# tczhangzhi/pytorch-distributed

Measured on NVIDIA H100. Metric: ResNet-50 images/sec (device-timed, max over ranks), higher is better.
Workload: dtype bf16; 1 GPU; model=resnet50, global_batch=256, image_size=224, parallelism=dp1, entry=distributed, comm=fused, nvls=False, channels_last=True, fused_bn=True, optimizer=fused, cuda_graph=True, l2_policy=inputs larger than L2 (4 x 38.5 MB bf16 batches + GBs of activations per step), overlap_optimizer=True, bucket_view=False, cudnn=deterministic

## Files before the change

### pytorch_distributed_b200/_ext.py

```python
from __future__ import annotations

import hashlib
import importlib.util
import os
import shutil
import sys
import threading

_HERE = os.path.dirname(os.path.abspath(__file__))
_CSRC = os.path.join(_HERE, "csrc")
_NAME = "_C"
_SO = os.path.join(_HERE, _NAME + ".so")
_STAMP = os.path.join(_HERE, _NAME + ".hash")
_SOURCES = ["bindings.cpp", "symm.cpp", "hvd_core.cpp", "collectives.cu", "optim.cu", "bn_act.cu", "data_ops.cu", "gemm_bnstats.cu", "stem_conv.cu",
            "resample.cu"]
_lock = threading.Lock()
_mod = None
_err = None

CUDA_FLAGS = ["-gencode", "arch=compute_90a,code=sm_90a", "-lineinfo", "-O3", "--use_fast_math", "-std=c++17",
              "--expt-relaxed-constexpr", "-Xptxas", "-v"]


def source_hash() -> str:
    h = hashlib.sha256()
    for fn in sorted(os.listdir(_CSRC)):
        if fn.endswith((".cu", ".cpp", ".h", ".cuh")):
            with open(os.path.join(_CSRC, fn), "rb") as f:
                h.update(fn.encode())
                h.update(f.read())
    h.update(" ".join(CUDA_FLAGS).encode())
    return h.hexdigest()


def is_built() -> bool:
    if not (os.path.exists(_SO) and os.path.exists(_STAMP)):
        return False
    with open(_STAMP) as f:
        return f.read().strip() == source_hash()


def build(verbose: bool = False, force: bool = False) -> str:
    with _lock:
        if is_built() and not force:
            return _SO
        from torch.utils import cpp_extension
        build_dir = os.path.join(_CSRC, "build")
        os.makedirs(build_dir, exist_ok=True)
        os.environ.setdefault("MAX_JOBS", str(max(2, min(8, (os.cpu_count() or 4)))))
        cpp_extension.load(
            name=_NAME,
            sources=[os.path.join(_CSRC, s) for s in _SOURCES],
            extra_cflags=["-O3", "-std=c++17"],
            extra_cuda_cflags=CUDA_FLAGS,
            extra_include_paths=[_CSRC],
            build_directory=build_dir,
            verbose=verbose,
            is_python_module=False,
        )
        built = os.path.join(build_dir, _NAME + ".so")
        shutil.copyfile(built, _SO + ".tmp")
        os.replace(_SO + ".tmp", _SO)
        with open(_STAMP, "w") as f:
            f.write(source_hash())
        return _SO


def _import_so():
    import torch
    spec = importlib.util.spec_from_file_location("pytorch_distributed_b200." + _NAME, _SO)
    mod = importlib.util.module_from_spec(spec)
    spec.loader.exec_module(mod)
    sys.modules["pytorch_distributed_b200." + _NAME] = mod
    return mod


def lib(build_if_missing: bool = True):
    global _mod, _err
    if _mod is not None:
        return _mod
    if _err is not None:
        raise _err
    try:
        if not is_built():
            if not build_if_missing or os.environ.get("PTD_NO_BUILD") == "1":
                raise RuntimeError("native extension is not built (run `python -c 'import __graft_entry__ as g; g.build()'`)")
            build()
        _mod = _import_so()
        return _mod
    except Exception as e:
        _err = RuntimeError("pytorch_distributed_b200 native extension unavailable: %s" % (e,))
        raise _err from e


def available() -> bool:
    try:
        lib()
        return True
    except Exception:
        return False


def require_on_cuda() -> None:
    import torch
    if torch.cuda.is_available():
        lib()


launches = 0


def note_launch(n: int = 1) -> None:
    global launches
    launches += n
```

### pytorch_distributed_b200/csrc/bindings.cpp

```cpp
#include <torch/extension.h>

#include "hvd_core.h"
#include "host.h"
#include "symm.h"

namespace py = pybind11;
using namespace ptd;

namespace {

at::Tensor arena_view(const std::shared_ptr<SymmArena>& a, int64_t rank, int64_t offset_bytes, int64_t numel, const std::string& dtype) {
  at::ScalarType st;
  if (dtype == "float32") st = at::kFloat;
  else if (dtype == "bfloat16") st = at::kBFloat16;
  else if (dtype == "float16") st = at::kHalf;
  else if (dtype == "int32") st = at::kInt;
  else if (dtype == "uint8") st = at::kByte;
  else throw std::runtime_error("unsupported arena view dtype " + dtype);
  const int64_t esz = (int64_t)c10::elementSize(st);
  TORCH_CHECK(offset_bytes >= 0 && offset_bytes + numel * esz <= a->bytes(), "arena view out of range");
  TORCH_CHECK(offset_bytes % esz == 0, "misaligned arena view");
  const int r = a->single_process() ? (int)rank : a->rank();
  void* p = reinterpret_cast<void*>(a->ptr(r) + offset_bytes);
  auto keep = a;
  return at::from_blob(p, {numel}, [keep](void*) {}, at::TensorOptions().dtype(st).device(at::kCUDA, (c10::DeviceIndex)a->device(r)));
}

}

PYBIND11_MODULE(TORCH_EXTENSION_NAME, m) {
  m.doc() = "pytorch_distributed_b200 native runtime (sm_90a)";
  m.attr("MAX_WORLD") = kMaxWorld;
  m.attr("MAX_BLOCKS") = kMaxBlocks;
  m.attr("MAX_CHANNELS") = kMaxChannels;
  m.attr("MAX_PTRS") = kMaxPtrs;
  m.attr("SIGNAL_PAD_BYTES") = (int64_t)sizeof(SignalPad);
  m.attr("SEG_BYTES") = (int64_t)sizeof(Seg);
  m.def("multicast_supported", &multicast_supported);

  py::class_<SymmArena, std::shared_ptr<SymmArena>>(m, "SymmArena")
      .def(py::init<int, int, int, int64_t>(), py::arg("device"), py::arg("rank"), py::arg("world"), py::arg("bytes"))
      .def_static("create_local", &SymmArena::create_local)
      .def_static("from_pointers", &SymmArena::from_pointers)
      .def("export_fd", &SymmArena::export_fd)
      .def("open_socket", &SymmArena::open_socket)
      .def("send_fd", &SymmArena::send_fd)
      .def("recv_fd", &SymmArena::recv_fd, py::call_guard<py::gil_scoped_release>())
      .def("map_peer", &SymmArena::map_peer)
      .def("mc_create", &SymmArena::mc_create)
      .def("mc_import", &SymmArena::mc_import)
      .def("mc_add_device", &SymmArena::mc_add_device)
      .def("mc_bind_and_map", &SymmArena::mc_bind_and_map)
      .def("disable_multicast", &SymmArena::disable_multicast)
      .def_property_readonly("rank", &SymmArena::rank)
      .def_property_readonly("world", &SymmArena::world)
      .def_property_readonly("bytes", &SymmArena::bytes)
      .def_property_readonly("mc_ptr", &SymmArena::mc_ptr)
      .def_property_readonly("multicast_candidate", &SymmArena::multicast_candidate)
      .def_property_readonly("has_multicast", &SymmArena::has_multicast)
      .def_property_readonly("mc_error", &SymmArena::mc_error)
      .def_property_readonly("single_process", &SymmArena::single_process)
      .def("ptr", &SymmArena::ptr)
      .def("device", &SymmArena::device, py::arg("r") = 0)
      .def("status", &SymmArena::status)
      .def("set_timeout_ms", &SymmArena::set_timeout_ms)
      .def("ll_seq_ptr", &SymmArena::ll_seq_ptr, py::arg("r") = 0)
      .def("view", [](std::shared_ptr<SymmArena> a, int64_t offset, int64_t numel, const std::string& dtype, int64_t rank) {
             return arena_view(a, rank, offset, numel, dtype);
           }, py::arg("offset_bytes"), py::arg("numel"), py::arg("dtype"), py::arg("rank") = 0)
      .def("launch_plan",
           [](std::shared_ptr<SymmArena> a, int channel, int as_rank, int kind, int wire_dtype, bool nvls, int grid, std::vector<at::Tensor> tensors,
              int64_t seg_begin_ptr, int64_t segs_ptr, int64_t data_off_bytes, int64_t block_elems, int64_t plan_calls_ptr, int64_t found_inf_ptr,
              double scale, bool writeback, int root, int flags, int64_t result_off_bytes) {
             launch_plan(a->ctx(channel, as_rank), kind, wire_dtype, nvls, grid, tensors, seg_begin_ptr, segs_ptr, data_off_bytes, block_elems,
                         plan_calls_ptr, found_inf_ptr, scale, writeback, root, flags, result_off_bytes);
           },
           py::arg("channel"), py::arg("as_rank"), py::arg("kind"), py::arg("wire_dtype"), py::arg("nvls"), py::arg("grid"), py::arg("tensors"),
           py::arg("seg_begin_ptr"), py::arg("segs_ptr"), py::arg("data_off_bytes"), py::arg("block_elems"), py::arg("plan_calls_ptr"),
           py::arg("found_inf_ptr"), py::arg("scale"), py::arg("writeback"), py::arg("root"), py::arg("flags") = 0,
           py::arg("result_off_bytes") = (int64_t)-1)
      .def("launch_barrier", [](std::shared_ptr<SymmArena> a, int channel) { launch_barrier(a->ctx(channel)); })
      .def("launch_metrics",
           [](std::shared_ptr<SymmArena> a, int channel, const at::Tensor& logits, const at::Tensor& target, c10::optional<at::Tensor> loss, at::Tensor out) {
             launch_metrics(a->ctx(channel), logits, target, loss, a->ll_seq_ptr(), out);
           })
      .def("launch_ll_allreduce", [](std::shared_ptr<SymmArena> a, int channel, const at::Tensor& in, at::Tensor out, double scale) {
        launch_ll_allreduce(a->ctx(channel), in, out, scale, a->ll_seq_ptr());
      });

  m.def("pack_pointers", &pack_pointers);
  m.def("fused_sgd_flat", &fused_sgd_flat, py::arg("grad"), py::arg("master"), py::arg("momentum"), py::arg("model_copy"), py::arg("hyper"),
        py::arg("found_inf"), py::arg("nesterov"), py::arg("first_step"));
  m.def("fused_sgd_multi", &fused_sgd_multi);
  m.def("multi_tensor_scale", &multi_tensor_scale);
  m.def("multi_tensor_axpby", &multi_tensor_axpby);
  m.def("amp_update_scale", &amp_update_scale);
  m.def("bn_act_forward", &bn_act_forward);
  m.def("bn_act_backward", &bn_act_backward);
  m.def("bn_act_backward2", &bn_act_backward2);
  m.def("stem_forward", &stem_forward);
  m.def("stem_forward_pre", &stem_forward_pre);
  m.def("stem_backward", &stem_backward);
  m.def("stem_im2col", &stem_im2col);
  m.def("conv1x1_bnstats", &conv1x1_bnstats);
  m.def("normalize_nhwc", &normalize_nhwc);
  m.def("resample_normalize", &resample_normalize, py::arg("arena"), py::arg("n"), py::arg("out_h"), py::arg("out_w"), py::arg("max_rows"),
        py::arg("a"), py::arg("b"), py::arg("out_dtype"), py::arg("channels_last"));
  m.def("p2p_copy_multi", &p2p_copy_multi);

  py::class_<FusionQueue, std::shared_ptr<FusionQueue>>(m, "FusionQueue")
      .def(py::init<int64_t, double, int64_t>(), py::arg("fusion_threshold_bytes"), py::arg("cycle_time_ms"), py::arg("cycle_bytes") = 0)
      .def("wait_idle", &FusionQueue::wait_idle, py::arg("timeout_ms"), py::call_guard<py::gil_scoped_release>())
      .def("wake", &FusionQueue::wake)
      .def("set_cycle_bytes", &FusionQueue::set_cycle_bytes)
      .def("cycle_bytes", &FusionQueue::cycle_bytes)
      .def("enable_timeline", &FusionQueue::enable_timeline)
      .def("timeline", &FusionQueue::timeline)
      .def("enqueue", &FusionQueue::enqueue, py::arg("name"), py::arg("nbytes"), py::arg("order_key"))
      .def("next_group", &FusionQueue::next_group, py::arg("timeout_ms"), py::call_guard<py::gil_scoped_release>())
      .def("flush", &FusionQueue::flush)
      .def("mark_done", &FusionQueue::mark_done)
      .def("wait", &FusionQueue::wait, py::arg("handle"), py::arg("timeout_ms"), py::call_guard<py::gil_scoped_release>())
      .def("pending", &FusionQueue::pending)
      .def("shutdown", &FusionQueue::shutdown)
      .def("stats", &FusionQueue::stats);
}
```

### pytorch_distributed_b200/csrc/bn_act.cu

```cuda
#include <ATen/cuda/CUDAContext.h>
#include <c10/cuda/CUDAGuard.h>
#include <torch/extension.h>

#include <map>

#include "common.cuh"
#include "host.h"

namespace ptd {

constexpr int kBnThreads = 256;
constexpr int kBnWarps = kBnThreads / 32;

struct RowMap {
  int cgs;
  int tpr;
  int rpp;
  int rlocal;
  int cg0;
  bool active;
  bool pow2;
};
__device__ __forceinline__ RowMap row_map(int C) {
  RowMap m;
  m.cgs = C >> 3;
  m.tpr = min(m.cgs, (int)blockDim.x);
  m.rpp = blockDim.x / m.tpr;
  m.rlocal = threadIdx.x / m.tpr;
  m.cg0 = threadIdx.x % m.tpr;
  m.active = m.rlocal < m.rpp;
  m.pow2 = (m.tpr & (m.tpr - 1)) == 0;
  return m;
}

__device__ __forceinline__ float ld_w(const void* p, int dt, int i) {
  switch (dt) {
    case kF32: return reinterpret_cast<const float*>(p)[i];
    case kBF16: return __bfloat162float(reinterpret_cast<const __nv_bfloat16*>(p)[i]);
    default: return __half2float(reinterpret_cast<const __half*>(p)[i]);
  }
}
__device__ __forceinline__ void st_w(void* p, int dt, int i, float v) {
  switch (dt) {
    case kF32: reinterpret_cast<float*>(p)[i] = v; break;
    case kBF16: reinterpret_cast<__nv_bfloat16*>(p)[i] = __float2bfloat16_rn(v); break;
    default: reinterpret_cast<__half*>(p)[i] = __float2half_rn(v); break;
  }
}

__device__ __forceinline__ void cta_combine(const RowMap& m, int cg_base, float (&a)[8], float (&b)[8], float* sm, float* part, int C) {
  const int lane = threadIdx.x & 31, warp = threadIdx.x >> 5;
  const int width = m.tpr * 8;
  int slots, slot;
  bool writer = m.active;
  if (m.pow2 && m.tpr < 32) {
    for (int o = m.tpr; o < 32; o <<= 1) {
#pragma unroll
      for (int k = 0; k < 8; ++k) {
        a[k] += __shfl_xor_sync(0xffffffffu, a[k], o);
        b[k] += __shfl_xor_sync(0xffffffffu, b[k], o);
      }
    }
    slots = kBnWarps;
    slot = warp;
    writer = lane < m.tpr;
  } else {
    slots = m.rpp;
    slot = m.rlocal;
  }
  __syncthreads();
  if (writer) {
    float* row = sm + (size_t)slot * 2 * width + m.cg0 * 8;
#pragma unroll
    for (int k = 0; k < 8; ++k) { row[k] = a[k]; row[width + k] = b[k]; }
  }
  __syncthreads();
  for (int i = threadIdx.x; i < 2 * width; i += blockDim.x) {
    float s = 0.f;
    for (int r = 0; r < slots; ++r) s += sm[(size_t)r * 2 * width + i];
    const int half = i >= width, c = cg_base * 8 + (i - half * width);
    if (c < C) part[(size_t)blockIdx.x * 2 * C + half * C + c] = s;
  }
}

__global__ void __launch_bounds__(1024) combine_partials_kernel(const float* __restrict__ part, int nblocks, int n,
                                                                float* __restrict__ gsum) {
  __shared__ float sm[32][33];
  const int tx = threadIdx.x & 31, ty = threadIdx.x >> 5;
  const int i = blockIdx.x * 32 + tx;
  float s = 0.f;
  if (i < n)
    for (int b = ty; b < nblocks; b += 32) s += part[(size_t)b * n + i];
  sm[ty][tx] = s;
  __syncthreads();
  if (ty == 0 && i < n) {
    float t = 0.f;
    for (int k = 0; k < 32; ++k) t += sm[k][tx];
    gsum[i] += t;
  }
}

void combine_partials(const float* part, int nblocks, int n, float* gsum, cudaStream_t st) {
  combine_partials_kernel<<<(n + 31) / 32, 1024, 0, st>>>(part, nblocks, n, gsum);
  C10_CUDA_KERNEL_LAUNCH_CHECK();
}

static at::Tensor partials(const at::Tensor& x, int grid, int C) {
  return at::empty({grid, 2 * C}, x.options().dtype(at::kFloat).memory_format(at::MemoryFormat::Contiguous));
}

template <typename T>
__global__ void __launch_bounds__(kBnThreads) bn_stats_kernel(const T* __restrict__ x, float* __restrict__ part, int64_t M, int C,
                                                              int rows_per_block) {
  extern __shared__ float sm[];
  const RowMap m = row_map(C);
  const int64_t r0 = (int64_t)blockIdx.x * rows_per_block, r1 = min(M, r0 + (int64_t)rows_per_block);
  for (int cgb = 0; cgb < m.cgs; cgb += m.tpr) {
    const int cg = cgb + m.cg0;
    float s[8], q[8];
#pragma unroll
    for (int k = 0; k < 8; ++k) { s[k] = 0.f; q[k] = 0.f; }
    if (m.active && cg < m.cgs) {
      const T* p = x + cg * 8;
      int64_t r = r0 + m.rlocal;
      for (; r + 7 * (int64_t)m.rpp < r1; r += 8 * (int64_t)m.rpp) {
        float f[8][8];
#pragma unroll
        for (int u = 0; u < 8; ++u) load8<T>(p + (r + (int64_t)u * m.rpp) * C, f[u]);
#pragma unroll
        for (int u = 0; u < 8; ++u)
#pragma unroll
          for (int k = 0; k < 8; ++k) { s[k] += f[u][k]; q[k] += f[u][k] * f[u][k]; }
      }
      for (; r < r1; r += m.rpp) {
        float f[8];
        load8<T>(p + r * C, f);
#pragma unroll
        for (int k = 0; k < 8; ++k) { s[k] += f[k]; q[k] += f[k] * f[k]; }
      }
    }
    cta_combine(m, cgb, s, q, sm, part, C);
  }
}

template <typename T, bool RELU, bool RES>
__global__ void __launch_bounds__(kBnThreads) bn_apply_kernel(const T* __restrict__ x, const T* __restrict__ res, T* __restrict__ y,
                                                              uint8_t* __restrict__ mask, const float* __restrict__ gsum,
                                                              const void* __restrict__ w, const void* __restrict__ b, int wdt,
                                                              float* __restrict__ running_mean, float* __restrict__ running_var,
                                                              int64_t* __restrict__ num_batches_tracked, float* __restrict__ saved,
                                                              int64_t M, int C, float eps, float momentum, int training) {
  const RowMap m = row_map(C);
  const float inv_m = 1.f / (float)M;
  if (training && num_batches_tracked && blockIdx.x == 0 && threadIdx.x == 0) *num_batches_tracked += 1;
  if (!m.active) return;
  for (int cg = m.cg0; cg < m.cgs; cg += m.tpr) {
    float sc[8], sh[8];
#pragma unroll
    for (int k = 0; k < 8; ++k) {
      const int c = cg * 8 + k;
      float mean, var;
      if (training) {
        mean = gsum[c] * inv_m;
        var = fmaxf(gsum[C + c] * inv_m - mean * mean, 0.f);
      } else {
        mean = running_mean[c];
        var = running_var[c];
      }
      const float invstd = rsqrtf(var + eps);
      sc[k] = ld_w(w, wdt, c) * invstd;
      sh[k] = ld_w(b, wdt, c) - mean * sc[k];
      if (training && blockIdx.x == 0 && m.rlocal == 0) {
        saved[c] = mean;
        saved[C + c] = invstd;
        if (running_mean) {
          const float unbiased = M > 1 ? var * ((float)M / (float)(M - 1)) : var;
          running_mean[c] = (1.f - momentum) * running_mean[c] + momentum * mean;
          running_var[c] = (1.f - momentum) * running_var[c] + momentum * unbiased;
        }
      }
    }
    const int64_t stride = (int64_t)gridDim.x * m.rpp;
    const int64_t coff = cg * 8;
    int64_t r = (int64_t)blockIdx.x * m.rpp + m.rlocal;
    for (; r + 3 * stride < M; r += 4 * stride) {
      float f[4][8], g[4][8];
#pragma unroll
      for (int u = 0; u < 4; ++u) load8<T>(x + (r + u * stride) * C + coff, f[u]);
      if constexpr (RES) {
#pragma unroll
        for (int u = 0; u < 4; ++u) load8<T>(res + (r + u * stride) * C + coff, g[u]);
      }
#pragma unroll
      for (int u = 0; u < 4; ++u) {
        unsigned bits = 0;
#pragma unroll
        for (int k = 0; k < 8; ++k) {
          float v = f[u][k] * sc[k] + sh[k];
          if constexpr (RES) v += g[u][k];
          if constexpr (RELU) { bits |= (v > 0.f ? 1u : 0u) << k; v = fmaxf(v, 0.f); }
          f[u][k] = v;
        }
        store8<T>(y + (r + u * stride) * C + coff, f[u]);
        if constexpr (RELU) { if (mask) mask[(r + u * stride) * m.cgs + cg] = (uint8_t)bits; }
      }
    }
    for (; r < M; r += stride) {
      float f[8], g[8];
      load8<T>(x + r * C + coff, f);
      if constexpr (RES) load8<T>(res + r * C + coff, g);
      unsigned bits = 0;
#pragma unroll
      for (int k = 0; k < 8; ++k) {
        float v = f[k] * sc[k] + sh[k];
        if constexpr (RES) v += g[k];
        if constexpr (RELU) { bits |= (v > 0.f ? 1u : 0u) << k; v = fmaxf(v, 0.f); }
        f[k] = v;
      }
      store8<T>(y + r * C + coff, f);
      if constexpr (RELU) { if (mask) mask[r * m.cgs + cg] = (uint8_t)bits; }
    }
  }
}

template <typename T, bool RELU>
__global__ void __launch_bounds__(kBnThreads) bn_bwd_reduce_kernel(const T* __restrict__ dy, const uint8_t* __restrict__ mask,
                                                                   const T* __restrict__ x, const float* __restrict__ saved,
                                                                   float* __restrict__ part, int64_t M, int C, int rows_per_block) {
  extern __shared__ float sm[];
  const RowMap m = row_map(C);
  const int64_t r0 = (int64_t)blockIdx.x * rows_per_block, r1 = min(M, r0 + (int64_t)rows_per_block);
  for (int cgb = 0; cgb < m.cgs; cgb += m.tpr) {
    const int cg = cgb + m.cg0;
    float s[8], q[8];
#pragma unroll
    for (int k = 0; k < 8; ++k) { s[k] = 0.f; q[k] = 0.f; }
    if (m.active && cg < m.cgs) {
      float mean[8];
#pragma unroll
      for (int k = 0; k < 8; ++k) mean[k] = saved[cg * 8 + k];
      const int64_t coff = cg * 8;
      int64_t r = r0 + m.rlocal;
      for (; r + 3 * (int64_t)m.rpp < r1; r += 4 * (int64_t)m.rpp) {
        float d[4][8], v[4][8];
        unsigned bits[4];
#pragma unroll
        for (int u = 0; u < 4; ++u) {
          const int64_t row = r + (int64_t)u * m.rpp;
          load8<T>(dy + row * C + coff, d[u]);
          load8<T>(x + row * C + coff, v[u]);
          if constexpr (RELU) bits[u] = mask[row * m.cgs + cg];
        }
#pragma unroll
        for (int u = 0; u < 4; ++u)
#pragma unroll
          for (int k = 0; k < 8; ++k) {
            float dz = d[u][k];
            if constexpr (RELU) dz = (bits[u] >> k) & 1u ? dz : 0.f;
            s[k] += dz;
            q[k] += dz * (v[u][k] - mean[k]);
          }
      }
      for (; r < r1; r += m.rpp) {
        float d[8], v[8];
        load8<T>(dy + r * C + coff, d);
        load8<T>(x + r * C + coff, v);
        unsigned bits = 0;
        if constexpr (RELU) bits = mask[r * m.cgs + cg];
#pragma unroll
        for (int k = 0; k < 8; ++k) {
          float dz = d[k];
          if constexpr (RELU) dz = (bits >> k) & 1u ? dz : 0.f;
          s[k] += dz;
          q[k] += dz * (v[k] - mean[k]);
        }
      }
#pragma unroll
      for (int k = 0; k < 8; ++k) q[k] *= saved[C + cg * 8 + k];
    }
    cta_combine(m, cgb, s, q, sm, part, C);
  }
}

template <typename T, bool RELU, bool RES>
__global__ void __launch_bounds__(kBnThreads) bn_bwd_apply_kernel(const T* __restrict__ dy, const uint8_t* __restrict__ mask,
                                                                  const T* __restrict__ x, const float* __restrict__ saved,
                                                                  const float* __restrict__ gsum, const void* __restrict__ w, int wdt,
                                                                  T* __restrict__ dx, T* __restrict__ dres, void* __restrict__ dw,
                                                                  void* __restrict__ db, int64_t M, int C) {
  const RowMap m = row_map(C);
  if (!m.active) return;
  const float inv_m = 1.f / (float)M;
  for (int cg = m.cg0; cg < m.cgs; cg += m.tpr) {
    float ka[8], kb[8], kd[8];
#pragma unroll
    for (int k = 0; k < 8; ++k) {
      const int c = cg * 8 + k;
      const float mean = saved[c], invstd = saved[C + c];
      const float sdz = gsum[c], sdzx = gsum[C + c];
      ka[k] = ld_w(w, wdt, c) * invstd;
      kb[k] = -ka[k] * invstd * sdzx * inv_m;
      kd[k] = -ka[k] * sdz * inv_m - kb[k] * mean;
      if (blockIdx.x == 0 && m.rlocal == 0) {
        st_w(dw, wdt, c, sdzx);
        st_w(db, wdt, c, sdz);
      }
    }
    const int64_t stride = (int64_t)gridDim.x * m.rpp;
    const int64_t coff = cg * 8;
    int64_t r = (int64_t)blockIdx.x * m.rpp + m.rlocal;
    for (; r + 3 * stride < M; r += 4 * stride) {
      float d[4][8], v[4][8];
      unsigned bits[4];
#pragma unroll
      for (int u = 0; u < 4; ++u) {
        const int64_t row = r + u * stride;
        load8<T>(dy + row * C + coff, d[u]);
        load8<T>(x + row * C + coff, v[u]);
        if constexpr (RELU) bits[u] = mask[row * m.cgs + cg];
      }
#pragma unroll
      for (int u = 0; u < 4; ++u) {
        const int64_t off = (r + u * stride) * C + coff;
#pragma unroll
        for (int k = 0; k < 8; ++k) {
          float dz = d[u][k];
          if constexpr (RELU) dz = (bits[u] >> k) & 1u ? dz : 0.f;
          d[u][k] = dz;
          v[u][k] = ka[k] * dz + kb[k] * v[u][k] + kd[k];
        }
        store8<T>(dx + off, v[u]);
        if constexpr (RES) store8<T>(dres + off, d[u]);
      }
    }
    for (; r < M; r += stride) {
      float d[8], v[8];
      const int64_t off = r * C + coff;
      load8<T>(dy + off, d);
      load8<T>(x + off, v);
      unsigned bits = 0;
      if constexpr (RELU) bits = mask[r * m.cgs + cg];
#pragma unroll
      for (int k = 0; k < 8; ++k) {
        float dz = d[k];
        if constexpr (RELU) dz = (bits >> k) & 1u ? dz : 0.f;
        d[k] = dz;
        v[k] = ka[k] * dz + kb[k] * v[k] + kd[k];
      }
      store8<T>(dx + off, v);
      if constexpr (RES) store8<T>(dres + off, d);
    }
  }
}

static int wdtype(const at::Tensor& t) {
  switch (t.scalar_type()) {
    case at::kFloat: return kF32;
    case at::kBFloat16: return kBF16;
    case at::kHalf: return kF16;
    default: TORCH_CHECK(false, "unsupported BN parameter dtype"); return 0;
  }
}

static void check_nhwc(const at::Tensor& t, const char* name) {
  TORCH_CHECK(t.is_cuda() && t.dim() == 4, name, " must be a 4-d CUDA tensor");
  TORCH_CHECK(t.is_contiguous(at::MemoryFormat::ChannelsLast), name, " must be channels_last contiguous");
}

struct Geometry { int64_t M; int C; int tpr; int rpp; int sms; size_t smem; };
static Geometry geometry(const at::Tensor& x) {
  Geometry g;
  g.C = (int)x.size(1);
  g.M = x.numel() / g.C;
  TORCH_CHECK(g.C % 8 == 0 && g.C <= 16384, "fused BN needs C % 8 == 0 and C <= 16384 (got ", g.C, ")");
  g.tpr = std::min(g.C / 8, kBnThreads);
  g.rpp = kBnThreads / g.tpr;
  g.sms = at::cuda::getCurrentDeviceProperties()->multiProcessorCount;
  const bool pow2 = (g.tpr & (g.tpr - 1)) == 0;
  const int slots = (pow2 && g.tpr < 32) ? kBnWarps : g.rpp;
  g.smem = (size_t)slots * 2 * g.tpr * 8 * sizeof(float);
  return g;
}
template <typename K>
static int resident_ctas(K kernel, size_t smem) {
  static std::map<std::pair<const void*, size_t>, int> cache;
  const auto key = std::make_pair(reinterpret_cast<const void*>(kernel), smem);
  auto it = cache.find(key);
  if (it != cache.end()) return it->second;
  int n = 1;
  if (cudaOccupancyMaxActiveBlocksPerMultiprocessor(&n, kernel, kBnThreads, smem) != cudaSuccess || n < 1) n = 1;
  cache[key] = n;
  return n;
}
static int reduce_grid(const Geometry& g, int* rows_per_block, int resident = 4) {
  int64_t blocks = (g.M + (int64_t)g.rpp * 8 - 1) / ((int64_t)g.rpp * 8);
  const int64_t wave = (int64_t)g.sms * resident;
  if (blocks > wave) blocks = blocks >= 2 * wave && g.M / (2 * wave) >= (int64_t)g.rpp * 64 ? 2 * wave : wave;
  blocks = std::max<int64_t>(blocks, 1);
  int64_t rpb = (g.M + blocks - 1) / blocks;
  rpb = (rpb + g.rpp - 1) / g.rpp * g.rpp;
  *rows_per_block = (int)rpb;
  return (int)((g.M + rpb - 1) / rpb);
}
static int apply_grid(const Geometry& g) {
  int64_t blocks = (g.M + (int64_t)g.rpp * 4 - 1) / ((int64_t)g.rpp * 4);
  return (int)std::max<int64_t>(std::min<int64_t>(blocks, (int64_t)g.sms * 8), 1);
}

template <typename T>
static void fwd_impl(const at::Tensor& x, const at::Tensor* res, at::Tensor& y, at::Tensor& mask, at::Tensor& work, at::Tensor& saved,
                     const at::Tensor& w, const at::Tensor& b, at::Tensor& rm, at::Tensor& rv, at::Tensor& nbt, bool training, float momentum,
                     float eps, bool relu, bool stats_ready) {
  const Geometry g = geometry(x);
  cudaStream_t st = at::cuda::getCurrentCUDAStream();
  const T* xp = reinterpret_cast<const T*>(x.data_ptr());
  T* yp = reinterpret_cast<T*>(y.data_ptr());
  const T* rp = res ? reinterpret_cast<const T*>(res->data_ptr()) : nullptr;
  float* wk = work.defined() ? work.data_ptr<float>() : nullptr;
  if (training && !stats_ready) {
    int rpb;
    const int grid = reduce_grid(g, &rpb, resident_ctas(bn_stats_kernel<T>, g.smem));
    at::Tensor part = partials(x, grid, g.C);
    bn_stats_kernel<T><<<grid, kBnThreads, g.smem, st>>>(xp, part.data_ptr<float>(), g.M, g.C, rpb);
    C10_CUDA_KERNEL_LAUNCH_CHECK();
    combine_partials(part.data_ptr<float>(), grid, 2 * g.C, wk, st);
  }
  const int grid = apply_grid(g);
  float* rmp = rm.defined() ? rm.data_ptr<float>() : nullptr;
  float* rvp = rv.defined() ? rv.data_ptr<float>() : nullptr;
  int64_t* nb = nbt.defined() ? nbt.data_ptr<int64_t>() : nullptr;
  float* sv = saved.defined() ? saved.data_ptr<float>() : nullptr;
  uint8_t* mk = mask.defined() ? mask.data_ptr<uint8_t>() : nullptr;
  const int wdt = wdtype(w);
#define APPLY(R, S) \
  bn_apply_kernel<T, R, S><<<grid, kBnThreads, 0, st>>>(xp, rp, yp, mk, wk, w.data_ptr(), b.data_ptr(), wdt, rmp, rvp, nb, sv, g.M, g.C, eps, momentum, training ? 1 : 0)
  if (relu) { if (res) APPLY(true, true); else APPLY(true, false); }
  else      { if (res) APPLY(false, true); else APPLY(false, false); }
#undef APPLY
  C10_CUDA_KERNEL_LAUNCH_CHECK();
}

std::vector<at::Tensor> bn_act_forward(const at::Tensor& x, const c10::optional<at::Tensor>& residual, const at::Tensor& weight,
                                       const at::Tensor& bias, at::Tensor running_mean, at::Tensor running_var,
                                       c10::optional<at::Tensor> num_batches_tracked, bool training, double momentum, double eps, bool relu,
                                       bool need_mask, at::Tensor work, bool stats_ready) {
  check_nhwc(x, "x");
  TORCH_CHECK(weight.scalar_type() == bias.scalar_type() && weight.is_contiguous() && bias.is_contiguous());
  if (running_mean.defined()) TORCH_CHECK(running_mean.scalar_type() == at::kFloat && running_var.scalar_type() == at::kFloat, "running stats must be fp32");
  TORCH_CHECK(training || running_mean.defined(), "eval mode needs running statistics");
  const at::Tensor* res = nullptr;
  if (residual.has_value() && residual->defined()) {
    check_nhwc(*residual, "residual");
    TORCH_CHECK(residual->sizes() == x.sizes() && residual->scalar_type() == x.scalar_type(), "residual must match x");
    res = &*residual;
  }
  c10::cuda::CUDAGuard guard(x.device());
  const int C = (int)x.size(1);
  at::Tensor y = at::empty_like(x, x.options().memory_format(at::MemoryFormat::ChannelsLast));
  at::Tensor saved, mask, nbt;
  if (num_batches_tracked.has_value() && num_batches_tracked->defined()) {
    nbt = *num_batches_tracked;
    TORCH_CHECK(nbt.scalar_type() == at::kLong && nbt.is_cuda());
  }
  if (training) {
    TORCH_CHECK(work.defined() && work.scalar_type() == at::kFloat && work.numel() >= 2 * C, "work buffer too small");
    saved = at::empty({2 * C}, x.options().dtype(at::kFloat));
  }
  if (relu && need_mask) mask = at::empty({x.numel() / 8}, x.options().dtype(at::kByte));
  switch (x.scalar_type()) {
    case at::kBFloat16: fwd_impl<__nv_bfloat16>(x, res, y, mask, work, saved, weight, bias, running_mean, running_var, nbt, training, (float)momentum, (float)eps, relu, stats_ready); break;
    case at::kHalf: fwd_impl<__half>(x, res, y, mask, work, saved, weight, bias, running_mean, running_var, nbt, training, (float)momentum, (float)eps, relu, stats_ready); break;
    case at::kFloat: fwd_impl<float>(x, res, y, mask, work, saved, weight, bias, running_mean, running_var, nbt, training, (float)momentum, (float)eps, relu, stats_ready); break;
    default: TORCH_CHECK(false, "unsupported activation dtype");
  }
  return {y, saved, mask};
}

template <typename T>
static void bwd_impl(const at::Tensor& dy, const at::Tensor& mask, const at::Tensor& x, const at::Tensor& saved, at::Tensor& work,
                     const at::Tensor& w, at::Tensor& dx, at::Tensor& dres, at::Tensor& dw, at::Tensor& db, bool relu, bool write_res) {
  const Geometry g = geometry(x);
  cudaStream_t st = at::cuda::getCurrentCUDAStream();
  const T* dyp = reinterpret_cast<const T*>(dy.data_ptr());
  const uint8_t* mk = relu ? mask.data_ptr<uint8_t>() : nullptr;
  const T* xp = reinterpret_cast<const T*>(x.data_ptr());
  float* wk = work.data_ptr<float>();
  const float* sv = saved.data_ptr<float>();
  int rpb;
  const int rgrid = reduce_grid(g, &rpb, relu ? resident_ctas(bn_bwd_reduce_kernel<T, true>, g.smem)
                                             : resident_ctas(bn_bwd_reduce_kernel<T, false>, g.smem));
  at::Tensor part = partials(x, rgrid, g.C);
  float* pp = part.data_ptr<float>();
  if (relu) bn_bwd_reduce_kernel<T, true><<<rgrid, kBnThreads, g.smem, st>>>(dyp, mk, xp, sv, pp, g.M, g.C, rpb);
  else      bn_bwd_reduce_kernel<T, false><<<rgrid, kBnThreads, g.smem, st>>>(dyp, mk, xp, sv, pp, g.M, g.C, rpb);
  C10_CUDA_KERNEL_LAUNCH_CHECK();
  combine_partials(pp, rgrid, 2 * g.C, wk, st);
  const int grid = apply_grid(g);
  T* dxp = reinterpret_cast<T*>(dx.data_ptr());
  T* drp = write_res ? reinterpret_cast<T*>(dres.data_ptr()) : nullptr;
  const int wdt = wdtype(w);
#define BAPPLY(R, S) \
  bn_bwd_apply_kernel<T, R, S><<<grid, kBnThreads, 0, st>>>(dyp, mk, xp, sv, wk, w.data_ptr(), wdt, dxp, drp, dw.data_ptr(), db.data_ptr(), g.M, g.C)
  if (relu) { if (write_res) BAPPLY(true, true); else BAPPLY(true, false); }
  else      { if (write_res) BAPPLY(false, true); else BAPPLY(false, false); }
#undef BAPPLY
  C10_CUDA_KERNEL_LAUNCH_CHECK();
}

std::vector<at::Tensor> bn_act_backward(const at::Tensor& dy_in, const at::Tensor& x, const c10::optional<at::Tensor>& mask_opt,
                                        const at::Tensor& weight, const at::Tensor& saved, bool relu, bool has_residual, at::Tensor work) {
  check_nhwc(x, "x");
  at::Tensor dy = dy_in.is_contiguous(at::MemoryFormat::ChannelsLast) ? dy_in : dy_in.contiguous(at::MemoryFormat::ChannelsLast);
  TORCH_CHECK(dy.scalar_type() == x.scalar_type() && dy.sizes() == x.sizes());
  at::Tensor mask;
  if (relu) {
    TORCH_CHECK(mask_opt.has_value() && mask_opt->defined() && mask_opt->scalar_type() == at::kByte && mask_opt->numel() == x.numel() / 8,
                "ReLU backward needs the forward's bit mask");
    mask = *mask_opt;
  }
  const int C = (int)x.size(1);
  TORCH_CHECK(work.defined() && work.scalar_type() == at::kFloat && work.numel() >= 2 * C, "work buffer too small");
  c10::cuda::CUDAGuard guard(x.device());
  at::Tensor dx = at::empty_like(x, x.options().memory_format(at::MemoryFormat::ChannelsLast));
  at::Tensor dres;
  if (has_residual) dres = (!relu) ? dy : at::empty_like(x, x.options().memory_format(at::MemoryFormat::ChannelsLast));
  at::Tensor dw = at::empty_like(weight), db = at::empty_like(weight);
  const bool write_res = has_residual && relu;
  switch (x.scalar_type()) {
    case at::kBFloat16: bwd_impl<__nv_bfloat16>(dy, mask, x, saved, work, weight, dx, dres, dw, db, relu, write_res); break;
    case at::kHalf: bwd_impl<__half>(dy, mask, x, saved, work, weight, dx, dres, dw, db, relu, write_res); break;
    case at::kFloat: bwd_impl<float>(dy, mask, x, saved, work, weight, dx, dres, dw, db, relu, write_res); break;
    default: TORCH_CHECK(false, "unsupported activation dtype");
  }
  return {dx, dres, dw, db};
}

template <typename T, bool RELU>
__global__ void __launch_bounds__(kBnThreads) bn_bwd_reduce_sum_kernel(const T* __restrict__ dya, const T* __restrict__ dyb,
                                                                       const uint8_t* __restrict__ mask, const T* __restrict__ x,
                                                                       const float* __restrict__ saved, T* __restrict__ gout,
                                                                       float* __restrict__ part, int64_t M, int C, int rows_per_block) {
  extern __shared__ float sm[];
  const RowMap m = row_map(C);
  const int64_t r0 = (int64_t)blockIdx.x * rows_per_block, r1 = min(M, r0 + (int64_t)rows_per_block);
  for (int cgb = 0; cgb < m.cgs; cgb += m.tpr) {
    const int cg = cgb + m.cg0;
    float s[8], q[8];
#pragma unroll
    for (int k = 0; k < 8; ++k) { s[k] = 0.f; q[k] = 0.f; }
    if (m.active && cg < m.cgs) {
      float mean[8];
#pragma unroll
      for (int k = 0; k < 8; ++k) mean[k] = saved[cg * 8 + k];
      const int64_t coff = cg * 8;
      int64_t r = r0 + m.rlocal;
      for (; r + (int64_t)m.rpp < r1; r += 2 * (int64_t)m.rpp) {
        float d[2][8], e[2][8], v[2][8];
        unsigned bits[2];
#pragma unroll
        for (int u = 0; u < 2; ++u) {
          const int64_t row = r + (int64_t)u * m.rpp;
          load8<T>(dya + row * C + coff, d[u]);
          load8<T>(dyb + row * C + coff, e[u]);
          load8<T>(x + row * C + coff, v[u]);
          if constexpr (RELU) bits[u] = mask[row * m.cgs + cg];
        }
#pragma unroll
        for (int u = 0; u < 2; ++u) {
#pragma unroll
          for (int k = 0; k < 8; ++k) {
            float dz = to_f32<T>(from_f32<T>(d[u][k] + e[u][k]));
            if constexpr (RELU) dz = (bits[u] >> k) & 1u ? dz : 0.f;
            d[u][k] = dz;
            s[k] += dz;
            q[k] += dz * (v[u][k] - mean[k]);
          }
          store8<T>(gout + (r + (int64_t)u * m.rpp) * C + coff, d[u]);
        }
      }
      for (; r < r1; r += m.rpp) {
        float d[8], e[8], v[8];
        load8<T>(dya + r * C + coff, d);
        load8<T>(dyb + r * C + coff, e);
        load8<T>(x + r * C + coff, v);
        unsigned bits = 0;
        if constexpr (RELU) bits = mask[r * m.cgs + cg];
#pragma unroll
        for (int k = 0; k < 8; ++k) {
          float dz = to_f32<T>(from_f32<T>(d[k] + e[k]));
          if constexpr (RELU) dz = (bits >> k) & 1u ? dz : 0.f;
          d[k] = dz;
          s[k] += dz;
          q[k] += dz * (v[k] - mean[k]);
        }
        store8<T>(gout + r * C + coff, d);
      }
#pragma unroll
      for (int k = 0; k < 8; ++k) q[k] *= saved[C + cg * 8 + k];
    }
    cta_combine(m, cgb, s, q, sm, part, C);
  }
}

template <typename T>
static void bwd2_impl(const at::Tensor& dya, const at::Tensor& dyb, const at::Tensor& mask, const at::Tensor& x, const at::Tensor& saved,
                      at::Tensor& work, const at::Tensor& w, at::Tensor& g_out, at::Tensor& dx, at::Tensor& dw, at::Tensor& db, bool relu) {
  const Geometry g = geometry(x);
  cudaStream_t st = at::cuda::getCurrentCUDAStream();
  const T* ap = reinterpret_cast<const T*>(dya.data_ptr());
  const T* bp = reinterpret_cast<const T*>(dyb.data_ptr());
  const uint8_t* mk = relu ? mask.data_ptr<uint8_t>() : nullptr;
  const T* xp = reinterpret_cast<const T*>(x.data_ptr());
  T* gp = reinterpret_cast<T*>(g_out.data_ptr());
  float* wk = work.data_ptr<float>();
  const float* sv = saved.data_ptr<float>();
  int rpb;
  const int rgrid = reduce_grid(g, &rpb, relu ? resident_ctas(bn_bwd_reduce_sum_kernel<T, true>, g.smem)
                                             : resident_ctas(bn_bwd_reduce_sum_kernel<T, false>, g.smem));
  at::Tensor part = partials(x, rgrid, g.C);
  float* pp = part.data_ptr<float>();
  if (relu) bn_bwd_reduce_sum_kernel<T, true><<<rgrid, kBnThreads, g.smem, st>>>(ap, bp, mk, xp, sv, gp, pp, g.M, g.C, rpb);
  else      bn_bwd_reduce_sum_kernel<T, false><<<rgrid, kBnThreads, g.smem, st>>>(ap, bp, mk, xp, sv, gp, pp, g.M, g.C, rpb);
  C10_CUDA_KERNEL_LAUNCH_CHECK();
  combine_partials(pp, rgrid, 2 * g.C, wk, st);
  bn_bwd_apply_kernel<T, false, false><<<apply_grid(g), kBnThreads, 0, st>>>(gp, nullptr, xp, sv, wk, w.data_ptr(), wdtype(w),
                                                                           reinterpret_cast<T*>(dx.data_ptr()), nullptr, dw.data_ptr(),
                                                                           db.data_ptr(), g.M, g.C);
  C10_CUDA_KERNEL_LAUNCH_CHECK();
}

std::vector<at::Tensor> bn_act_backward2(const at::Tensor& dy_a_in, const at::Tensor& dy_b_in, const at::Tensor& x,
                                         const c10::optional<at::Tensor>& mask_opt, const at::Tensor& weight, const at::Tensor& saved,
                                         bool relu, at::Tensor work) {
  check_nhwc(x, "x");
  const auto cl = at::MemoryFormat::ChannelsLast;
  at::Tensor dya = dy_a_in.is_contiguous(cl) ? dy_a_in : dy_a_in.contiguous(cl);
  at::Tensor dyb = dy_b_in.is_contiguous(cl) ? dy_b_in : dy_b_in.contiguous(cl);
  TORCH_CHECK(dya.scalar_type() == x.scalar_type() && dya.sizes() == x.sizes() && dya.device() == x.device(), "dy_a must match x");
  TORCH_CHECK(dyb.scalar_type() == x.scalar_type() && dyb.sizes() == x.sizes() && dyb.device() == x.device(), "dy_b must match x");
  at::Tensor mask;
  if (relu) {
    TORCH_CHECK(mask_opt.has_value() && mask_opt->defined() && mask_opt->scalar_type() == at::kByte && mask_opt->numel() == x.numel() / 8,
                "ReLU backward needs the forward's bit mask");
    mask = *mask_opt;
  }
  const int C = (int)x.size(1);
  TORCH_CHECK(work.defined() && work.scalar_type() == at::kFloat && work.numel() >= 2 * C, "work buffer too small");
  TORCH_CHECK(saved.defined() && saved.scalar_type() == at::kFloat && saved.numel() >= 2 * C, "saved statistics missing");
  c10::cuda::CUDAGuard guard(x.device());
  at::Tensor g = at::empty_like(x, x.options().memory_format(cl));
  at::Tensor dx = at::empty_like(x, x.options().memory_format(cl));
  at::Tensor dw = at::empty_like(weight), db = at::empty_like(weight);
  switch (x.scalar_type()) {
    case at::kBFloat16: bwd2_impl<__nv_bfloat16>(dya, dyb, mask, x, saved, work, weight, g, dx, dw, db, relu); break;
    case at::kHalf: bwd2_impl<__half>(dya, dyb, mask, x, saved, work, weight, g, dx, dw, db, relu); break;
    case at::kFloat: bwd2_impl<float>(dya, dyb, mask, x, saved, work, weight, g, dx, dw, db, relu); break;
    default: TORCH_CHECK(false, "unsupported activation dtype");
  }
  return {dx, g, dw, db};
}

}

namespace ptd {

struct PoolGeom { int H, W, OH, OW; };

__device__ __forceinline__ void stem_scale_shift(const float* gsum, const float* rm, const float* rv, const void* w, const void* b, int wdt,
                                                 int cg, int C, float inv_m, float eps, int training, float (&sc)[8], float (&sh)[8],
                                                 float (&mean)[8], float (&var)[8]) {
#pragma unroll
  for (int k = 0; k < 8; ++k) {
    const int c = cg * 8 + k;
    if (training) {
      mean[k] = gsum[c] * inv_m;
      var[k] = fmaxf(gsum[C + c] * inv_m - mean[k] * mean[k], 0.f);
    } else {
      mean[k] = rm[c];
      var[k] = rv[c];
    }
    const float invstd = rsqrtf(var[k] + eps);
    sc[k] = ld_w(w, wdt, c) * invstd;
    sh[k] = ld_w(b, wdt, c) - mean[k] * sc[k];
  }
}

template <typename T>
__global__ void __launch_bounds__(kBnThreads) stem_fwd_kernel(const T* __restrict__ x, T* __restrict__ y, uint2* __restrict__ code,
                                                              const float* __restrict__ gsum, const void* __restrict__ w,
                                                              const void* __restrict__ b, int wdt, float* __restrict__ running_mean,
                                                              float* __restrict__ running_var, int64_t* __restrict__ nbt,
                                                              float* __restrict__ saved, int64_t M, int N, int C, PoolGeom g, float eps,
                                                              float momentum, int training) {
  const int cgs = C >> 3;
  const int cg = threadIdx.x % cgs;
  float sc[8], sh[8], mean[8], var[8];
  stem_scale_shift(gsum, running_mean, running_var, w, b, wdt, cg, C, 1.f / (float)M, eps, training, sc, sh, mean, var);
  if (training && blockIdx.x == 0 && threadIdx.x < cgs) {
    if (threadIdx.x == 0 && nbt) *nbt += 1;
#pragma unroll
    for (int k = 0; k < 8; ++k) {
      const int c = cg * 8 + k;
      saved[c] = mean[k];
      saved[C + c] = rsqrtf(var[k] + eps);
      if (running_mean) {
        const float unbiased = M > 1 ? var[k] * ((float)M / (float)(M - 1)) : var[k];
        running_mean[c] = (1.f - momentum) * running_mean[c] + momentum * mean[k];
        running_var[c] = (1.f - momentum) * running_var[c] + momentum * unbiased;
      }
    }
  }
  const int64_t total = (int64_t)N * g.OH * g.OW;
  const int ppb = blockDim.x / cgs;
  for (int p = blockIdx.x * ppb + threadIdx.x / cgs; p < (int)total; p += gridDim.x * ppb) {
    const int ow = p % g.OW;
    const int t_ = p / g.OW;
    const int oh = t_ % g.OH;
    const int64_t n = t_ / g.OH;
    float best[8];
    uint32_t sel[8];
#pragma unroll
    for (int k = 0; k < 8; ++k) { best[k] = 0.f; sel[k] = 15u; }
    const T* base = x + n * g.H * g.W * C + cg * 8;
#pragma unroll
    for (int kh = 0; kh < 3; ++kh) {
      const int ih = 2 * oh - 1 + kh;
      if (ih < 0 || ih >= g.H) continue;
#pragma unroll
      for (int kw = 0; kw < 3; ++kw) {
        const int iw = 2 * ow - 1 + kw;
        if (iw < 0 || iw >= g.W) continue;
        float f[8];
        load8<T>(base + ((int64_t)ih * g.W + iw) * C, f);
#pragma unroll
        for (int k = 0; k < 8; ++k) {
          const float v = f[k] * sc[k] + sh[k];
          if (v > best[k]) { best[k] = v; sel[k] = (uint32_t)(kh * 3 + kw); }
        }
      }
    }
    store8<T>(y + (int64_t)p * C + cg * 8, best);
    if (code) {
      uint2 word;
      word.x = sel[0] | (sel[1] << 8) | (sel[2] << 16) | (sel[3] << 24);
      word.y = sel[4] | (sel[5] << 8) | (sel[6] << 16) | (sel[7] << 24);
      code[(int64_t)p * cgs + cg] = word;
    }
  }
}

template <typename T> struct Pair;
template <> struct Pair<__nv_bfloat16> {
  using P = __nv_bfloat162;
  static __device__ __forceinline__ uint32_t add(uint32_t a, uint32_t b) {
    P r = __hadd2(*reinterpret_cast<P*>(&a), *reinterpret_cast<P*>(&b));
    return *reinterpret_cast<uint32_t*>(&r);
  }
  static __device__ __forceinline__ float2 widen(uint32_t a) { return __bfloat1622float2(*reinterpret_cast<P*>(&a)); }
};
template <> struct Pair<__half> {
  using P = __half2;
  static __device__ __forceinline__ uint32_t add(uint32_t a, uint32_t b) {
    P r = __hadd2(*reinterpret_cast<P*>(&a), *reinterpret_cast<P*>(&b));
    return *reinterpret_cast<uint32_t*>(&r);
  }
  static __device__ __forceinline__ float2 widen(uint32_t a) { return __half22float2(*reinterpret_cast<P*>(&a)); }
};

template <typename T>
__device__ __forceinline__ void stem_gather_dz(const T* __restrict__ dp, const uint2* __restrict__ code, int64_t n, int ih, int iw, int cg,
                                               int cgs, int C, const PoolGeom& g, float (&dz)[8]) {
  const int oh0 = ih >> 1, oh1 = min((ih + 1) >> 1, g.OH - 1);
  const int ow0 = iw >> 1, ow1 = min((iw + 1) >> 1, g.OW - 1);
  if constexpr (sizeof(T) == 2) {
    uint32_t a0 = 0, a1 = 0, a2 = 0, a3 = 0;
    for (int oh = oh0; oh <= oh1; ++oh) {
      const int kh = ih - (2 * oh - 1);
      for (int ow = ow0; ow <= ow1; ++ow) {
        const uint32_t pat = (uint32_t)(kh * 3 + iw - (2 * ow - 1)) * 0x01010101u;
        const int64_t p = (n * g.OH + oh) * g.OW + ow;
        const uint2 cw = code[p * cgs + cg];
        const V4 d = ld_stream(dp + p * C + cg * 8);
        const uint32_t m0 = __vcmpeq4(cw.x, pat), m1 = __vcmpeq4(cw.y, pat);
        a0 = Pair<T>::add(a0, d.x & __byte_perm(m0, 0, 0x1100));
        a1 = Pair<T>::add(a1, d.y & __byte_perm(m0, 0, 0x3322));
        a2 = Pair<T>::add(a2, d.z & __byte_perm(m1, 0, 0x1100));
        a3 = Pair<T>::add(a3, d.w & __byte_perm(m1, 0, 0x3322));
      }
    }
    float2 t;
    t = Pair<T>::widen(a0); dz[0] = t.x; dz[1] = t.y;
    t = Pair<T>::widen(a1); dz[2] = t.x; dz[3] = t.y;
    t = Pair<T>::widen(a2); dz[4] = t.x; dz[5] = t.y;
    t = Pair<T>::widen(a3); dz[6] = t.x; dz[7] = t.y;
  } else {
#pragma unroll
    for (int k = 0; k < 8; ++k) dz[k] = 0.f;
    for (int oh = oh0; oh <= oh1; ++oh) {
      const int kh = ih - (2 * oh - 1);
      for (int ow = ow0; ow <= ow1; ++ow) {
        const uint32_t want = (uint32_t)(kh * 3 + iw - (2 * ow - 1));
        const int64_t p = (n * g.OH + oh) * g.OW + ow;
        const uint2 cw = code[p * cgs + cg];
        float d[8];
        load8<T>(dp + p * C + cg * 8, d);
#pragma unroll
        for (int k = 0; k < 8; ++k) {
          const uint32_t sel = ((k < 4 ? cw.x : cw.y) >> (8 * (k & 3))) & 255u;
          dz[k] += sel == want ? d[k] : 0.f;
        }
      }
    }
  }
}

template <typename T>
struct QuadDz {
  uint32_t a[4][4];
  __device__ __forceinline__ void clear() {
#pragma unroll
    for (int i = 0; i < 4; ++i)
#pragma unroll
      for (int j = 0; j < 4; ++j) a[i][j] = 0u;
  }
  __device__ __forceinline__ void hit(int pos, const uint2& cw, const V4& d, uint32_t want) {
    const uint32_t pat = want * 0x01010101u;
    const uint32_t m0 = __vcmpeq4(cw.x, pat), m1 = __vcmpeq4(cw.y, pat);
    a[pos][0] = Pair<T>::add(a[pos][0], d.x & __byte_perm(m0, 0, 0x1100));
    a[pos][1] = Pair<T>::add(a[pos][1], d.y & __byte_perm(m0, 0, 0x3322));
    a[pos][2] = Pair<T>::add(a[pos][2], d.z & __byte_perm(m1, 0, 0x1100));
    a[pos][3] = Pair<T>::add(a[pos][3], d.w & __byte_perm(m1, 0, 0x3322));
  }
  __device__ __forceinline__ void widen(int pos, float (&dz)[8]) const {
    float2 t;
    t = Pair<T>::widen(a[pos][0]); dz[0] = t.x; dz[1] = t.y;
    t = Pair<T>::widen(a[pos][1]); dz[2] = t.x; dz[3] = t.y;
    t = Pair<T>::widen(a[pos][2]); dz[4] = t.x; dz[5] = t.y;
    t = Pair<T>::widen(a[pos][3]); dz[6] = t.x; dz[7] = t.y;
  }
};

template <typename T>
__device__ __forceinline__ void stem_quad_dz(const T* __restrict__ dp, const uint2* __restrict__ code, int64_t n, int k, int j, int cg, int cgs,
                                             int C, const PoolGeom& g, QuadDz<T>& qd) {
  qd.clear();
  const bool has_r = (j + 1) < g.OW, has_b = (k + 1) < g.OH;
  const int64_t pA = (n * g.OH + k) * g.OW + j;
  {
    const uint2 cw = code[pA * cgs + cg];
    const V4 d = ld_stream(dp + pA * C + cg * 8);
    qd.hit(0, cw, d, 4u); qd.hit(1, cw, d, 5u); qd.hit(2, cw, d, 7u); qd.hit(3, cw, d, 8u);
  }
  if (has_r) {
    const uint2 cw = code[(pA + 1) * cgs + cg];
    const V4 d = ld_stream(dp + (pA + 1) * C + cg * 8);
    qd.hit(1, cw, d, 3u); qd.hit(3, cw, d, 6u);
  }
  if (has_b) {
    const int64_t pC = pA + g.OW;
    const uint2 cw = code[pC * cgs + cg];
    const V4 d = ld_stream(dp + pC * C + cg * 8);
    qd.hit(2, cw, d, 1u); qd.hit(3, cw, d, 2u);
    if (has_r) {
      const uint2 cw2 = code[(pC + 1) * cgs + cg];
      const V4 d2 = ld_stream(dp + (pC + 1) * C + cg * 8);
      qd.hit(3, cw2, d2, 0u);
    }
  }
}

template <typename T>
__global__ void __launch_bounds__(kBnThreads, 4) stem_bwd_reduce_kernel(const T* __restrict__ dp, const uint2* __restrict__ code,
                                                                     const T* __restrict__ x, const float* __restrict__ saved,
                                                                     float* __restrict__ part, int64_t M, int C, PoolGeom g,
                                                                     int rows_per_block) {
  extern __shared__ float sm[];
  const RowMap m = row_map(C);
  const int cg = m.cg0;
  const int QH = (g.H + 1) >> 1, QW = (g.W + 1) >> 1;
  const int nrows = (int)(M / ((int64_t)g.H * g.W)) * QH;
  const int row0 = blockIdx.x * rows_per_block, row1 = min(nrows, row0 + rows_per_block);
  float s[8], q[8], mean[8];
#pragma unroll
  for (int k = 0; k < 8; ++k) { s[k] = 0.f; q[k] = 0.f; mean[k] = saved[cg * 8 + k]; }
  for (int row = row0; row < row1; ++row) {
    const int n = row / QH, k = row - n * QH;
    for (int j = m.rlocal; j < QW; j += m.rpp) {
      if constexpr (sizeof(T) == 2) {
        QuadDz<T> qd;
        stem_quad_dz<T>(dp, code, n, k, j, cg, m.cgs, C, g, qd);
#pragma unroll
        for (int pos = 0; pos < 4; ++pos) {
          const int ih = 2 * k + (pos >> 1), iw = 2 * j + (pos & 1);
          if (ih < g.H && iw < g.W) {
            float dz[8], v[8];
            qd.widen(pos, dz);
            load8<T>(x + (((int64_t)n * g.H + ih) * g.W + iw) * C + cg * 8, v);
#pragma unroll
            for (int c = 0; c < 8; ++c) { s[c] += dz[c]; q[c] += dz[c] * (v[c] - mean[c]); }
          }
        }
      } else {
#pragma unroll
        for (int pos = 0; pos < 4; ++pos) {
          const int ih = 2 * k + (pos >> 1), iw = 2 * j + (pos & 1);
          if (ih < g.H && iw < g.W) {
            float dz[8], v[8];
            stem_gather_dz<T>(dp, code, n, ih, iw, cg, m.cgs, C, g, dz);
            load8<T>(x + (((int64_t)n * g.H + ih) * g.W + iw) * C + cg * 8, v);
#pragma unroll
            for (int c = 0; c < 8; ++c) { s[c] += dz[c]; q[c] += dz[c] * (v[c] - mean[c]); }
          }
        }
      }
    }
  }
#pragma unroll
  for (int k = 0; k < 8; ++k) q[k] *= saved[C + cg * 8 + k];
  cta_combine(m, 0, s, q, sm, part, C);
}

template <typename T>
__global__ void __launch_bounds__(kBnThreads, 4) stem_bwd_apply_kernel(const T* __restrict__ dp, const uint2* __restrict__ code,
                                                                    const T* __restrict__ x, const float* __restrict__ saved,
                                                                    const float* __restrict__ gsum, const void* __restrict__ w, int wdt,
                                                                    T* __restrict__ dx, void* __restrict__ dw, void* __restrict__ db,
                                                                    int64_t M, int C, PoolGeom g, int rows_per_block) {
  const RowMap m = row_map(C);
  const int cg = m.cg0;
  const float inv_m = 1.f / (float)M;
  float ka[8], kb[8], kd[8];
#pragma unroll
  for (int k = 0; k < 8; ++k) {
    const int c = cg * 8 + k;
    const float mean = saved[c], invstd = saved[C + c];
    const float sdz = gsum[c], sdzx = gsum[C + c];
    ka[k] = ld_w(w, wdt, c) * invstd;
    kb[k] = -ka[k] * invstd * sdzx * inv_m;
    kd[k] = -ka[k] * sdz * inv_m - kb[k] * mean;
    if (blockIdx.x == 0 && m.rlocal == 0) {
      st_w(dw, wdt, c, sdzx);
      st_w(db, wdt, c, sdz);
    }
  }
  const int QH = (g.H + 1) >> 1, QW = (g.W + 1) >> 1;
  const int nrows = (int)(M / ((int64_t)g.H * g.W)) * QH;
  const int row0 = blockIdx.x * rows_per_block, row1 = min(nrows, row0 + rows_per_block);
  for (int row = row0; row < row1; ++row) {
    const int n = row / QH, k = row - n * QH;
    for (int j = m.rlocal; j < QW; j += m.rpp) {
      QuadDz<T> qd;
      if constexpr (sizeof(T) == 2) stem_quad_dz<T>(dp, code, n, k, j, cg, m.cgs, C, g, qd);
#pragma unroll
      for (int pos = 0; pos < 4; ++pos) {
        const int ih = 2 * k + (pos >> 1), iw = 2 * j + (pos & 1);
        if (ih < g.H && iw < g.W) {
          float dz[8], v[8];
          if constexpr (sizeof(T) == 2) qd.widen(pos, dz);
          else stem_gather_dz<T>(dp, code, n, ih, iw, cg, m.cgs, C, g, dz);
          const int64_t off = (((int64_t)n * g.H + ih) * g.W + iw) * C + cg * 8;
          load8<T>(x + off, v);
#pragma unroll
          for (int c = 0; c < 8; ++c) v[c] = ka[c] * dz[c] + kb[c] * v[c] + kd[c];
          store8<T>(dx + off, v);
        }
      }
    }
  }
}

static PoolGeom pool_geom(const at::Tensor& x) {
  PoolGeom g;
  g.H = (int)x.size(2);
  g.W = (int)x.size(3);
  g.OH = (g.H + 2 - 3) / 2 + 1;
  g.OW = (g.W + 2 - 3) / 2 + 1;
  return g;
}

template <typename T>
static void stem_fwd_impl(const at::Tensor& x, at::Tensor& y, at::Tensor& code, at::Tensor& work, at::Tensor& saved, const at::Tensor& w,
                          const at::Tensor& b, at::Tensor& rm, at::Tensor& rv, at::Tensor& nbt, bool training, float momentum, float eps,
                          bool stats_ready) {
  const Geometry g = geometry(x);
  const PoolGeom pg = pool_geom(x);
  cudaStream_t st = at::cuda::getCurrentCUDAStream();
  const T* xp = reinterpret_cast<const T*>(x.data_ptr());
  float* wk = work.defined() ? work.data_ptr<float>() : nullptr;
  if (training && !stats_ready) {
    int rpb;
    const int grid = reduce_grid(g, &rpb, resident_ctas(bn_stats_kernel<T>, g.smem));
    at::Tensor part = partials(x, grid, g.C);
    bn_stats_kernel<T><<<grid, kBnThreads, g.smem, st>>>(xp, part.data_ptr<float>(), g.M, g.C, rpb);
    C10_CUDA_KERNEL_LAUNCH_CHECK();
    combine_partials(part.data_ptr<float>(), grid, 2 * g.C, wk, st);
  }
  const int cgs = g.C / 8;
  const int64_t total = x.size(0) * pg.OH * pg.OW;
  const int ppb = kBnThreads / cgs;
  const int grid = (int)std::max<int64_t>(1, std::min<int64_t>((total + ppb - 1) / ppb, (int64_t)g.sms * 16));
  stem_fwd_kernel<T><<<grid, kBnThreads, 0, st>>>(xp, reinterpret_cast<T*>(y.data_ptr()),
                                                 code.defined() ? reinterpret_cast<uint2*>(code.data_ptr()) : nullptr, wk, w.data_ptr(),
                                                 b.data_ptr(), wdtype(w), rm.defined() ? rm.data_ptr<float>() : nullptr,
                                                 rv.defined() ? rv.data_ptr<float>() : nullptr, nbt.defined() ? nbt.data_ptr<int64_t>() : nullptr,
                                                 saved.defined() ? saved.data_ptr<float>() : nullptr, g.M, (int)x.size(0), g.C, pg, eps, momentum,
                                                 training ? 1 : 0);
  C10_CUDA_KERNEL_LAUNCH_CHECK();
}

static std::vector<at::Tensor> stem_forward_common(const at::Tensor& x, const at::Tensor& weight, const at::Tensor& bias,
                                                   at::Tensor running_mean, at::Tensor running_var,
                                                   c10::optional<at::Tensor> num_batches_tracked, bool training, double momentum, double eps,
                                                   bool need_code, at::Tensor work, bool stats_ready) {
  check_nhwc(x, "x");
  const int C = (int)x.size(1);
  TORCH_CHECK(C % 8 == 0 && kBnThreads % (C / 8) == 0, "fused stem needs C/8 to divide ", kBnThreads);
  TORCH_CHECK(x.numel() / C < (int64_t)1 << 30, "fused stem: too many pixels for 32-bit indexing");
  TORCH_CHECK(training || running_mean.defined(), "eval mode needs running statistics");
  c10::cuda::CUDAGuard guard(x.device());
  const PoolGeom pg = pool_geom(x);
  at::Tensor y = at::empty({x.size(0), C, pg.OH, pg.OW}, x.options().memory_format(at::MemoryFormat::ChannelsLast));
  at::Tensor saved, code, nbt;
  if (num_batches_tracked.has_value() && num_batches_tracked->defined()) nbt = *num_batches_tracked;
  if (training) {
    TORCH_CHECK(work.defined() && work.numel() >= 2 * C, "work buffer too small");
    saved = at::empty({2 * C}, x.options().dtype(at::kFloat));
  }
  if (need_code) code = at::empty({y.numel()}, x.options().dtype(at::kByte));
  switch (x.scalar_type()) {
    case at::kBFloat16: stem_fwd_impl<__nv_bfloat16>(x, y, code, work, saved, weight, bias, running_mean, running_var, nbt, training, (float)momentum, (float)eps, stats_ready); break;
    case at::kHalf: stem_fwd_impl<__half>(x, y, code, work, saved, weight, bias, running_mean, running_var, nbt, training, (float)momentum, (float)eps, stats_ready); break;
    case at::kFloat: stem_fwd_impl<float>(x, y, code, work, saved, weight, bias, running_mean, running_var, nbt, training, (float)momentum, (float)eps, stats_ready); break;
    default: TORCH_CHECK(false, "unsupported activation dtype");
  }
  return {y, saved, code};
}

std::vector<at::Tensor> stem_forward(const at::Tensor& x, const at::Tensor& weight, const at::Tensor& bias, at::Tensor running_mean,
                                     at::Tensor running_var, c10::optional<at::Tensor> num_batches_tracked, bool training, double momentum,
                                     double eps, bool need_code, at::Tensor work) {
  return stem_forward_common(x, weight, bias, running_mean, running_var, num_batches_tracked, training, momentum, eps, need_code, work, false);
}
std::vector<at::Tensor> stem_forward_pre(const at::Tensor& x, const at::Tensor& weight, const at::Tensor& bias, at::Tensor running_mean,
                                         at::Tensor running_var, c10::optional<at::Tensor> num_batches_tracked, bool training, double momentum,
                                         double eps, bool need_code, at::Tensor work) {
  return stem_forward_common(x, weight, bias, running_mean, running_var, num_batches_tracked, training, momentum, eps, need_code, work, true);
}

template <typename T>
static void stem_bwd_impl(const at::Tensor& dp, const at::Tensor& code, const at::Tensor& x, const at::Tensor& saved, at::Tensor& work,
                          const at::Tensor& w, at::Tensor& dx, at::Tensor& dw, at::Tensor& db) {
  const Geometry g = geometry(x);
  const PoolGeom pg = pool_geom(x);
  cudaStream_t st = at::cuda::getCurrentCUDAStream();
  const T* dpp = reinterpret_cast<const T*>(dp.data_ptr());
  const uint2* cp = reinterpret_cast<const uint2*>(code.data_ptr());
  const T* xp = reinterpret_cast<const T*>(x.data_ptr());
  const int nrows = (int)(x.size(0) * ((pg.H + 1) / 2));
  const int rpb = std::max(1, std::min(4, nrows / (g.sms * 8)));
  const int grid = (nrows + rpb - 1) / rpb;
  at::Tensor part = partials(x, grid, g.C);
  stem_bwd_reduce_kernel<T><<<grid, kBnThreads, g.smem, st>>>(dpp, cp, xp, saved.data_ptr<float>(), part.data_ptr<float>(), g.M, g.C, pg, rpb);
  C10_CUDA_KERNEL_LAUNCH_CHECK();
  combine_partials(part.data_ptr<float>(), grid, 2 * g.C, work.data_ptr<float>(), st);
  stem_bwd_apply_kernel<T><<<grid, kBnThreads, 0, st>>>(dpp, cp, xp, saved.data_ptr<float>(), work.data_ptr<float>(), w.data_ptr(), wdtype(w),
                                                       reinterpret_cast<T*>(dx.data_ptr()), dw.data_ptr(), db.data_ptr(), g.M, g.C, pg, rpb);
  C10_CUDA_KERNEL_LAUNCH_CHECK();
}

std::vector<at::Tensor> stem_backward(const at::Tensor& dp_in, const at::Tensor& x, const at::Tensor& code, const at::Tensor& weight,
                                      const at::Tensor& saved, at::Tensor work) {
  check_nhwc(x, "x");
  at::Tensor dp = dp_in.is_contiguous(at::MemoryFormat::ChannelsLast) ? dp_in : dp_in.contiguous(at::MemoryFormat::ChannelsLast);
  const int C = (int)x.size(1);
  TORCH_CHECK(dp.scalar_type() == x.scalar_type() && dp.size(1) == C && code.scalar_type() == at::kByte && code.numel() == dp.numel());
  TORCH_CHECK(work.defined() && work.numel() >= 2 * C, "work buffer too small");
  c10::cuda::CUDAGuard guard(x.device());
  at::Tensor dx = at::empty_like(x, x.options().memory_format(at::MemoryFormat::ChannelsLast));
  at::Tensor dw = at::empty_like(weight), db = at::empty_like(weight);
  switch (x.scalar_type()) {
    case at::kBFloat16: stem_bwd_impl<__nv_bfloat16>(dp, code, x, saved, work, weight, dx, dw, db); break;
    case at::kHalf: stem_bwd_impl<__half>(dp, code, x, saved, work, weight, dx, dw, db); break;
    case at::kFloat: stem_bwd_impl<float>(dp, code, x, saved, work, weight, dx, dw, db); break;
    default: TORCH_CHECK(false, "unsupported activation dtype");
  }
  return {dx, dw, db};
}

}
```

### pytorch_distributed_b200/csrc/gemm_bnstats.cu

```cuda
#include <ATen/cuda/CUDAContext.h>
#include <c10/cuda/CUDAGuard.h>
#include <cuda.h>
#include <torch/extension.h>

#include "common.cuh"
#include "host.h"

namespace ptd {

constexpr int kBlockM = 128;
constexpr int kBlockK = 64;
constexpr int kConsumerThreads = 256;
constexpr int kGemmThreads = kConsumerThreads + 32;

template <int BLOCK_N> struct GemmCfg {
  static constexpr int kStages = BLOCK_N == 256 ? 3 : 4;
  static constexpr int kABytes = kBlockM * kBlockK * 2;
  static constexpr int kBBytes = BLOCK_N * kBlockK * 2;
  static constexpr int kCBytes = kBlockM * BLOCK_N * 2;
  static constexpr int kStatFloats = 2 * 4 * 128;
  static constexpr int kSmem = 1024 + kStages * (kABytes + kBBytes) + kCBytes + kStatFloats * 4 + 2 * kStages * 8;
};

__device__ __forceinline__ uint32_t smem_u32(const void* p) { return (uint32_t)__cvta_generic_to_shared(p); }

__device__ __forceinline__ void mbar_init(uint64_t* bar, uint32_t count) {
  asm volatile("mbarrier.init.shared::cta.b64 [%0], %1;" ::"r"(smem_u32(bar)), "r"(count));
}
__device__ __forceinline__ void mbar_expect_tx(uint64_t* bar, uint32_t bytes) {
  asm volatile("mbarrier.arrive.expect_tx.shared::cta.b64 _, [%0], %1;" ::"r"(smem_u32(bar)), "r"(bytes) : "memory");
}
__device__ __forceinline__ void mbar_arrive(uint64_t* bar) {
  asm volatile("mbarrier.arrive.shared::cta.b64 _, [%0];" ::"r"(smem_u32(bar)) : "memory");
}
__device__ __forceinline__ void mbar_wait(uint64_t* bar, uint32_t parity) {
  const uint32_t addr = smem_u32(bar);
  uint32_t done, spins = 0;
  do {
    asm volatile("{\n\t.reg .pred p;\n\tmbarrier.try_wait.parity.shared::cta.b64 p, [%1], %2;\n\tselp.u32 %0, 1, 0, p;\n\t}"
                 : "=r"(done) : "r"(addr), "r"(parity) : "memory");
    if (!done && ++spins > (1u << 24)) __trap();
  } while (!done);
}
__device__ __forceinline__ void tma_load_2d(void* smem_dst, const CUtensorMap* map, uint64_t* bar, int c0, int c1) {
  asm volatile("cp.async.bulk.tensor.2d.shared::cluster.global.mbarrier::complete_tx::bytes [%0], [%1, {%3, %4}], [%2];"
               ::"r"(smem_u32(smem_dst)), "l"(map), "r"(smem_u32(bar)), "r"(c0), "r"(c1) : "memory");
}
__device__ __forceinline__ void named_barrier(int id, int threads) {
  asm volatile("bar.sync %0, %1;" ::"r"(id), "r"(threads) : "memory");
}

__device__ __forceinline__ uint64_t gmma_desc(const void* smem_tile) {
  const uint64_t addr = (uint64_t)(smem_u32(smem_tile) >> 4) & 0x3FFFull;
  return addr | (1ull << 16) | ((uint64_t)(1024 >> 4) << 32) | (1ull << 62);
}

#define PTD_F8(i) "+f"(d[i]), "+f"(d[i + 1]), "+f"(d[i + 2]), "+f"(d[i + 3]), "+f"(d[i + 4]), "+f"(d[i + 5]), "+f"(d[i + 6]), "+f"(d[i + 7])

__device__ __forceinline__ void wgmma_n64(float* d, uint64_t adesc, uint64_t bdesc, int accumulate) {
  asm volatile(
      "{\n\t.reg .pred p;\n\tsetp.ne.b32 p, %34, 0;\n\t"
      "wgmma.mma_async.sync.aligned.m64n64k16.f32.bf16.bf16 "
      "{%0, %1, %2, %3, %4, %5, %6, %7, %8, %9, %10, %11, %12, %13, %14, %15, "
      "%16, %17, %18, %19, %20, %21, %22, %23, %24, %25, %26, %27, %28, %29, %30, %31}, %32, %33, p, 1, 1, 0, 0;\n\t}"
      : PTD_F8(0), PTD_F8(8), PTD_F8(16), PTD_F8(24)
      : "l"(adesc), "l"(bdesc), "r"(accumulate));
}
__device__ __forceinline__ void wgmma_n128(float* d, uint64_t adesc, uint64_t bdesc, int accumulate) {
  asm volatile(
      "{\n\t.reg .pred p;\n\tsetp.ne.b32 p, %66, 0;\n\t"
      "wgmma.mma_async.sync.aligned.m64n128k16.f32.bf16.bf16 "
      "{%0, %1, %2, %3, %4, %5, %6, %7, %8, %9, %10, %11, %12, %13, %14, %15, "
      "%16, %17, %18, %19, %20, %21, %22, %23, %24, %25, %26, %27, %28, %29, %30, %31, "
      "%32, %33, %34, %35, %36, %37, %38, %39, %40, %41, %42, %43, %44, %45, %46, %47, "
      "%48, %49, %50, %51, %52, %53, %54, %55, %56, %57, %58, %59, %60, %61, %62, %63}, %64, %65, p, 1, 1, 0, 0;\n\t}"
      : PTD_F8(0), PTD_F8(8), PTD_F8(16), PTD_F8(24), PTD_F8(32), PTD_F8(40), PTD_F8(48), PTD_F8(56)
      : "l"(adesc), "l"(bdesc), "r"(accumulate));
}
#undef PTD_F8

template <int N> __device__ __forceinline__ void fence_regs(float (&d)[N]) {
#pragma unroll
  for (int i = 0; i < N; ++i) asm volatile("" : "+f"(d[i])::"memory");
}

template <int BLOCK_N>
__global__ void __launch_bounds__(kGemmThreads, 1) gemm_bnstats_kernel(const __grid_constant__ CUtensorMap tmap_a,
                                                                       const __grid_constant__ CUtensorMap tmap_b,
                                                                       const __grid_constant__ CUtensorMap tmap_c,
                                                                       float* __restrict__ part, int N, int K, int m_tiles,
                                                                       int n_tiles, int ctas_per_n) {
  using Cfg = GemmCfg<BLOCK_N>;
  constexpr int kStages = Cfg::kStages;
  constexpr int kInstN = BLOCK_N >= 128 ? 128 : 64;
  constexpr int kBoxes = BLOCK_N / 64;
  extern __shared__ uint8_t smem_raw[];
  uint8_t* smem = reinterpret_cast<uint8_t*>((reinterpret_cast<uintptr_t>(smem_raw) + 1023) & ~(uintptr_t)1023);
  uint8_t* smem_a = smem;
  uint8_t* smem_b = smem_a + kStages * Cfg::kABytes;
  uint8_t* smem_c = smem_b + kStages * Cfg::kBBytes;
  float* smem_stats = reinterpret_cast<float*>(smem_c + Cfg::kCBytes);
  uint64_t* full_bar = reinterpret_cast<uint64_t*>(smem_stats + Cfg::kStatFloats);
  uint64_t* empty_bar = full_bar + kStages;

  const int warp = threadIdx.x >> 5, lane = threadIdx.x & 31;
  const int n_tile = blockIdx.x % n_tiles;
  const int m_first = blockIdx.x / n_tiles;
  const int n0 = n_tile * BLOCK_N;
  const int num_kb = K / kBlockK;

  if (threadIdx.x == 0) {
    for (int s = 0; s < kStages; ++s) { mbar_init(&full_bar[s], 1); mbar_init(&empty_bar[s], kConsumerThreads / 32); }
    asm volatile("fence.mbarrier_init.release.cluster;" ::: "memory");
  }
  __syncthreads();

  if (warp == kConsumerThreads / 32) {
    if (lane == 0) {
      asm volatile("prefetch.tensormap [%0];" ::"l"(&tmap_a) : "memory");
      asm volatile("prefetch.tensormap [%0];" ::"l"(&tmap_b) : "memory");
      uint32_t it = 0;
      for (int mt = m_first; mt < m_tiles; mt += ctas_per_n) {
        for (int kb = 0; kb < num_kb; ++kb, ++it) {
          const int s = it % kStages;
          mbar_wait(&empty_bar[s], ((it / kStages) & 1) ^ 1);
          mbar_expect_tx(&full_bar[s], Cfg::kABytes + Cfg::kBBytes);
          tma_load_2d(smem_a + s * Cfg::kABytes, &tmap_a, &full_bar[s], kb * kBlockK, mt * kBlockM);
          tma_load_2d(smem_b + s * Cfg::kBBytes, &tmap_b, &full_bar[s], kb * kBlockK, n0);
        }
      }
    }
    return;
  }

  const int wg = warp >> 2, t = threadIdx.x & 127, w = warp & 3;
  uint8_t* stg = smem_c + wg * (Cfg::kCBytes / 2);
  float acc[BLOCK_N / 2] = {};
  const int r0 = 16 * w + (lane >> 2);
  constexpr int kPairs = BLOCK_N / 2, kParts = 128 / kPairs, kRows = 64 / kParts;
  const int p = t % kPairs, rpart = t / kPairs;
  const int p_box = p >> 5, p_gran = (p & 31) >> 2, p_byte = (p & 3) * 4;
  float s0 = 0.f, s1 = 0.f, q0 = 0.f, q1 = 0.f;

  uint32_t it = 0;
  for (int mt = m_first; mt < m_tiles; mt += ctas_per_n) {
    for (int kb = 0; kb < num_kb; ++kb, ++it) {
      const int s = it % kStages;
      mbar_wait(&full_bar[s], (it / kStages) & 1);
      const uint64_t adesc = gmma_desc(smem_a + s * Cfg::kABytes + wg * 64 * 128);
      const uint64_t bdesc = gmma_desc(smem_b + s * Cfg::kBBytes);
      fence_regs(acc);
      asm volatile("wgmma.fence.sync.aligned;" ::: "memory");
#pragma unroll
      for (int k = 0; k < kBlockK / 16; ++k) {
#pragma unroll
        for (int h = 0; h < BLOCK_N / kInstN; ++h) {
          if constexpr (kInstN == 128) wgmma_n128(acc + h * 64, adesc + 2 * k, bdesc + h * 8 * kInstN + 2 * k, (kb | k) != 0);
          else wgmma_n64(acc + h * 32, adesc + 2 * k, bdesc + h * 8 * kInstN + 2 * k, (kb | k) != 0);
        }
      }
      asm volatile("wgmma.commit_group.sync.aligned;" ::: "memory");
      asm volatile("wgmma.wait_group.sync.aligned 0;" ::: "memory");
      fence_regs(acc);
      if (lane == 0) mbar_arrive(&empty_bar[s]);
    }

    if (t == 0) asm volatile("cp.async.bulk.wait_group.read 0;" ::: "memory");
    named_barrier(1 + wg, 128);
#pragma unroll
    for (int j = 0; j < BLOCK_N / 8; ++j) {
      uint8_t* box = stg + (j >> 3) * 8192 + (lane & 3) * 4;
      const int g = j & 7;
      *reinterpret_cast<uint32_t*>(box + r0 * 128 + ((g ^ (r0 & 7)) << 4)) = Wire<__nv_bfloat16>::pack2(acc[4 * j], acc[4 * j + 1]);
      *reinterpret_cast<uint32_t*>(box + (r0 + 8) * 128 + ((g ^ (r0 & 7)) << 4)) =
          Wire<__nv_bfloat16>::pack2(acc[4 * j + 2], acc[4 * j + 3]);
    }
    asm volatile("fence.proxy.async.shared::cta;" ::: "memory");
    named_barrier(1 + wg, 128);
    if (t == 0) {
#pragma unroll
      for (int b = 0; b < kBoxes; ++b)
        asm volatile("cp.async.bulk.tensor.2d.global.shared::cta.bulk_group [%0, {%2, %3}], [%1];"
                     ::"l"(&tmap_c), "r"(smem_u32(stg + b * 8192)), "r"(n0 + b * 64), "r"(mt * kBlockM + wg * 64) : "memory");
      asm volatile("cp.async.bulk.commit_group;" ::: "memory");
    }
    const uint8_t* src = stg + p_box * 8192 + p_byte;
#pragma unroll 8
    for (int r = rpart * kRows; r < rpart * kRows + kRows; ++r) {
      const float2 f = Wire<__nv_bfloat16>::unpack2(*reinterpret_cast<const uint32_t*>(src + r * 128 + ((p_gran ^ (r & 7)) << 4)));
      s0 += f.x; q0 += f.x * f.x;
      s1 += f.y; q1 += f.y * f.y;
    }
  }
  if (t == 0) asm volatile("cp.async.bulk.wait_group 0;" ::: "memory");
  float* my = smem_stats + wg * 4 * 128 + t;
  my[0] = s0; my[128] = s1; my[256] = q0; my[384] = q1;
  named_barrier(3, kConsumerThreads);
  for (int i = threadIdx.x; i < 2 * BLOCK_N; i += kConsumerThreads) {
    const int half = i >= BLOCK_N, col = i - half * BLOCK_N;
    const int pair = col >> 1, which = half * 2 + (col & 1);
    float v = 0.f;
    for (int w2 = 0; w2 < 2; ++w2)
      for (int pt = 0; pt < kParts; ++pt) v += smem_stats[w2 * 4 * 128 + which * 128 + pt * kPairs + pair];
    part[(size_t)m_first * 2 * N + half * N + n0 + col] = v;
  }
}

typedef CUresult (*EncodeTiledFn)(CUtensorMap*, CUtensorMapDataType, cuuint32_t, void*, const cuuint64_t*, const cuuint64_t*, const cuuint32_t*,
                                  const cuuint32_t*, CUtensorMapInterleave, CUtensorMapSwizzle, CUtensorMapL2promotion, CUtensorMapFloatOOBfill);

static EncodeTiledFn encode_fn() {
  static EncodeTiledFn fn = nullptr;
  if (!fn) {
    void* p = nullptr;
    cudaDriverEntryPointQueryResult q;
    TORCH_CHECK(cudaGetDriverEntryPoint("cuTensorMapEncodeTiled", &p, cudaEnableDefault, &q) == cudaSuccess && p, "cuTensorMapEncodeTiled not found");
    fn = reinterpret_cast<EncodeTiledFn>(p);
  }
  return fn;
}

static CUtensorMap make_map(const void* ptr, int64_t rows, int64_t cols, int box_rows, CUtensorMapL2promotion promo) {
  CUtensorMap m;
  cuuint64_t dims[2] = {(cuuint64_t)cols, (cuuint64_t)rows};
  cuuint64_t strides[1] = {(cuuint64_t)cols * 2};
  cuuint32_t box[2] = {(cuuint32_t)kBlockK, (cuuint32_t)box_rows};
  cuuint32_t estr[2] = {1, 1};
  CUresult r = encode_fn()(&m, CU_TENSOR_MAP_DATA_TYPE_BFLOAT16, 2, const_cast<void*>(ptr), dims, strides, box, estr, CU_TENSOR_MAP_INTERLEAVE_NONE,
                           CU_TENSOR_MAP_SWIZZLE_128B, promo, CU_TENSOR_MAP_FLOAT_OOB_FILL_NONE);
  TORCH_CHECK(r == CUDA_SUCCESS, "cuTensorMapEncodeTiled failed: ", (int)r);
  return m;
}

template <int BLOCK_N>
static void launch_gemm(const at::Tensor& a, const at::Tensor& b, at::Tensor& c, at::Tensor& gsum, int M, int N, int K) {
  constexpr int smem = GemmCfg<BLOCK_N>::kSmem;
  static bool configured[64] = {};
  const int dev = a.get_device();
  if (!configured[dev & 63]) {
    C10_CUDA_CHECK(cudaFuncSetAttribute(gemm_bnstats_kernel<BLOCK_N>, cudaFuncAttributeMaxDynamicSharedMemorySize, smem));
    configured[dev & 63] = true;
  }
  const CUtensorMap ma = make_map(a.data_ptr(), M, K, kBlockM, CU_TENSOR_MAP_L2_PROMOTION_L2_256B);
  const CUtensorMap mb = make_map(b.data_ptr(), N, K, BLOCK_N, CU_TENSOR_MAP_L2_PROMOTION_L2_256B);
  const CUtensorMap mc = make_map(c.data_ptr(), M, N, 64, CU_TENSOR_MAP_L2_PROMOTION_NONE);
  const int m_tiles = (M + kBlockM - 1) / kBlockM, n_tiles = N / BLOCK_N;
  const int sms = at::cuda::getCurrentDeviceProperties()->multiProcessorCount;
  const int ctas_per_n = std::max(1, std::min(m_tiles, sms / n_tiles));
  const int grid = ctas_per_n * n_tiles;
  cudaStream_t st = at::cuda::getCurrentCUDAStream();
  at::Tensor part = at::empty({ctas_per_n, 2 * N}, gsum.options());
  gemm_bnstats_kernel<BLOCK_N><<<grid, kGemmThreads, smem, st>>>(ma, mb, mc, part.data_ptr<float>(), N, K, m_tiles, n_tiles, ctas_per_n);
  C10_CUDA_KERNEL_LAUNCH_CHECK();
  combine_partials(part.data_ptr<float>(), ctas_per_n, 2 * N, gsum.data_ptr<float>(), st);
}

at::Tensor conv1x1_bnstats(const at::Tensor& x, const at::Tensor& weight, at::Tensor gsum) {
  TORCH_CHECK(x.is_cuda() && x.dim() == 4 && x.scalar_type() == at::kBFloat16 && x.is_contiguous(at::MemoryFormat::ChannelsLast),
              "conv1x1_bnstats: x must be a channels_last bf16 CUDA tensor");
  TORCH_CHECK(weight.dim() == 4 && weight.size(2) == 1 && weight.size(3) == 1 && weight.scalar_type() == at::kBFloat16, "weight must be [N, K, 1, 1] bf16");
  const int64_t M64 = x.size(0) * x.size(2) * x.size(3);
  const int K = (int)x.size(1), N = (int)weight.size(0);
  TORCH_CHECK(weight.size(1) == K && K % kBlockK == 0 && N % 64 == 0 && M64 < (int64_t)1 << 31, "conv1x1_bnstats: unsupported shape");
  TORCH_CHECK(gsum.scalar_type() == at::kFloat && gsum.numel() >= 2 * N && gsum.is_contiguous());
  TORCH_CHECK((reinterpret_cast<uintptr_t>(x.data_ptr()) & 15) == 0, "x must be 16-byte aligned");
  c10::cuda::CUDAGuard guard(x.device());
  at::Tensor w2 = weight.reshape({N, K}).contiguous();
  at::Tensor y = at::empty({x.size(0), N, x.size(2), x.size(3)}, x.options().memory_format(at::MemoryFormat::ChannelsLast));
  const int M = (int)M64;
  static const int max_bn = getenv("PTD_GEMM_BLOCK_N") ? atoi(getenv("PTD_GEMM_BLOCK_N")) : 256;
  if (N % 256 == 0 && max_bn >= 256) launch_gemm<256>(x, w2, y, gsum, M, N, K);
  else if (N % 128 == 0 && max_bn >= 128) launch_gemm<128>(x, w2, y, gsum, M, N, K);
  else launch_gemm<64>(x, w2, y, gsum, M, N, K);
  return y;
}

}
```

### pytorch_distributed_b200/csrc/host.h

```cpp
#pragma once
#include <cuda_runtime_api.h>
#include <torch/extension.h>

#include <cstdint>
#include <string>
#include <vector>

#include "comm_types.h"

namespace ptd {

struct Seg {
  int32_t tensor;
  int32_t len;
  int64_t src_off;
  int64_t arena_off;
};
static_assert(sizeof(Seg) == 24, "Seg layout is mirrored by numpy in parallel/plan.py");

void launch_plan(const CommCtx& ctx, int kind, int wire_dtype, bool nvls, int grid, const std::vector<at::Tensor>& tensors,
                 int64_t seg_begin_ptr, int64_t segs_ptr, int64_t data_off_bytes, int64_t block_elems, int64_t plan_calls_ptr,
                 int64_t found_inf_ptr, double scale, bool writeback, int root, int flags = 0, int64_t result_off_bytes = -1);
at::Tensor pack_pointers(const std::vector<at::Tensor>& tensors);
void launch_barrier(const CommCtx& ctx);
void launch_metrics(const CommCtx& ctx, const at::Tensor& logits, const at::Tensor& target, const c10::optional<at::Tensor>& loss,
                    int64_t ll_seq_ptr, at::Tensor out);
void launch_ll_allreduce(const CommCtx& ctx, const at::Tensor& in, at::Tensor out, double scale, int64_t ll_seq_ptr);

void fused_sgd_flat(at::Tensor grad, at::Tensor master, at::Tensor momentum, c10::optional<at::Tensor> model_copy,
                    at::Tensor hyper, c10::optional<at::Tensor> found_inf, bool nesterov, bool first_step);
void fused_sgd_multi(std::vector<at::Tensor> grads, std::vector<at::Tensor> params, std::vector<at::Tensor> momenta,
                     std::vector<at::Tensor> model_copies, at::Tensor hyper, c10::optional<at::Tensor> found_inf, bool nesterov,
                     bool first_step);
void multi_tensor_scale(std::vector<at::Tensor> src, std::vector<at::Tensor> dst, double scale, at::Tensor found_inf);
void multi_tensor_axpby(std::vector<at::Tensor> x, std::vector<at::Tensor> y, std::vector<at::Tensor> out, double a, double b,
                        at::Tensor found_inf);
void amp_update_scale(at::Tensor scale, at::Tensor growth_tracker, at::Tensor found_inf, double growth, double backoff,
                      int64_t interval, at::Tensor hyper);

void combine_partials(const float* part, int nblocks, int n, float* gsum, cudaStream_t st);
std::vector<at::Tensor> bn_act_forward(const at::Tensor& x, const c10::optional<at::Tensor>& residual, const at::Tensor& weight,
                                       const at::Tensor& bias, at::Tensor running_mean, at::Tensor running_var,
                                       c10::optional<at::Tensor> num_batches_tracked, bool training, double momentum, double eps, bool relu,
                                       bool need_mask, at::Tensor work, bool stats_ready);
std::vector<at::Tensor> bn_act_backward(const at::Tensor& dy, const at::Tensor& x, const c10::optional<at::Tensor>& mask,
                                        const at::Tensor& weight, const at::Tensor& saved, bool relu, bool has_residual, at::Tensor work);
std::vector<at::Tensor> bn_act_backward2(const at::Tensor& dy_a, const at::Tensor& dy_b, const at::Tensor& x,
                                         const c10::optional<at::Tensor>& mask, const at::Tensor& weight, const at::Tensor& saved, bool relu,
                                         at::Tensor work);

std::vector<at::Tensor> stem_forward(const at::Tensor& x, const at::Tensor& weight, const at::Tensor& bias, at::Tensor running_mean,
                                     at::Tensor running_var, c10::optional<at::Tensor> num_batches_tracked, bool training, double momentum,
                                     double eps, bool need_code, at::Tensor work);
std::vector<at::Tensor> stem_forward_pre(const at::Tensor& x, const at::Tensor& weight, const at::Tensor& bias, at::Tensor running_mean,
                                         at::Tensor running_var, c10::optional<at::Tensor> num_batches_tracked, bool training, double momentum,
                                         double eps, bool need_code, at::Tensor work);
std::vector<at::Tensor> stem_backward(const at::Tensor& dp, const at::Tensor& x, const at::Tensor& code, const at::Tensor& weight,
                                      const at::Tensor& saved, at::Tensor work);

at::Tensor conv1x1_bnstats(const at::Tensor& x, const at::Tensor& weight, at::Tensor gsum);

at::Tensor stem_im2col(const at::Tensor& x);

at::Tensor normalize_nhwc(const at::Tensor& src, const at::Tensor& mean, const at::Tensor& std, int64_t out_dtype, bool channels_last);

void p2p_copy_multi(std::vector<at::Tensor> src, std::vector<at::Tensor> dst, int64_t run_device);

at::Tensor resample_normalize(const at::Tensor& arena, int64_t n, int64_t out_h, int64_t out_w, int64_t max_rows, const at::Tensor& a,
                              const at::Tensor& b, int64_t out_dtype, bool channels_last);

}
```

### pytorch_distributed_b200/models/resnet.py

```python
from __future__ import annotations

import torch
import torch.nn as nn

from ..ops.bn_act import begin_step, bn_act
from ..ops.conv_bn import conv1x1_bn_act
from ..ops.stem import bn_relu_maxpool
from ..ops.stem_conv import can_use_stem_gemm, stem_conv_bn_relu_maxpool

import os as _os
FUSED_CONV1X1 = _os.environ.get("PTD_FUSED_CONV1X1", "1") == "1"
SPLIT_RESGRAD = _os.environ.get("PTD_SPLIT_RESGRAD", "1") == "1"
STEM_GEMM = _os.environ.get("PTD_STEM_GEMM", "1") == "1"


def _pair(x):
    return x if isinstance(x, tuple) else (x, x)


class BNAct(nn.BatchNorm2d):

    def __init__(self, num_features, relu=True, fused=None, **kw):
        super().__init__(num_features, **kw)
        self.relu = relu
        self.fused = fused

    def forward(self, x, residual=None, split=False):
        training = self.training or not self.track_running_stats
        nbt = self.num_batches_tracked if (self.training and self.track_running_stats) else None
        return bn_act(x, self.weight, self.bias, self.running_mean, self.running_var, residual=residual, relu=self.relu,
                      training=training, momentum=0.1 if self.momentum is None else self.momentum, eps=self.eps, fused=self.fused,
                      num_batches_tracked=nbt, split=split)


def _conv3x3(cin, cout, stride=1, groups=1, dilation=1):
    return nn.Conv2d(cin, cout, 3, stride=stride, padding=dilation, groups=groups, bias=False, dilation=dilation)


def _conv1x1(cin, cout, stride=1):
    return nn.Conv2d(cin, cout, 1, stride=stride, bias=False)


class _Downsample(nn.Sequential):

    def __init__(self, cin, cout, stride, fused):
        super().__init__(_conv1x1(cin, cout, stride), BNAct(cout, relu=False, fused=fused))

    def forward(self, x):
        return conv1x1_bn_act(x, self[0], self[1], enabled=FUSED_CONV1X1)


class BasicBlock(nn.Module):
    expansion = 1

    def __init__(self, cin, planes, stride=1, downsample=None, groups=1, base_width=64, fused=None):
        super().__init__()
        if groups != 1 or base_width != 64:
            raise ValueError("BasicBlock only supports groups=1 and base_width=64")
        self.conv1 = _conv3x3(cin, planes, stride)
        self.bn1 = BNAct(planes, relu=True, fused=fused)
        self.conv2 = _conv3x3(planes, planes)
        self.bn2 = BNAct(planes, relu=True, fused=fused)
        self.downsample = downsample
        self.stride = stride

    def forward(self, x):
        x, skip = _pair(x)
        identity = skip if self.downsample is None else self.downsample(skip)
        out = self.bn1(self.conv1(x))
        return self.bn2(self.conv2(out), identity, split=SPLIT_RESGRAD and self.training)


class Bottleneck(nn.Module):
    expansion = 4

    def __init__(self, cin, planes, stride=1, downsample=None, groups=1, base_width=64, fused=None):
        super().__init__()
        width = int(planes * (base_width / 64.0)) * groups
        self.conv1 = _conv1x1(cin, width)
        self.bn1 = BNAct(width, relu=True, fused=fused)
        self.conv2 = _conv3x3(width, width, stride, groups)
        self.bn2 = BNAct(width, relu=True, fused=fused)
        self.conv3 = _conv1x1(width, planes * self.expansion)
        self.bn3 = BNAct(planes * self.expansion, relu=True, fused=fused)
        self.downsample = downsample
        self.stride = stride

    def forward(self, x):
        x, skip = _pair(x)
        identity = skip if self.downsample is None else self.downsample(skip)
        out = conv1x1_bn_act(x, self.conv1, self.bn1, enabled=FUSED_CONV1X1)
        out = self.bn2(self.conv2(out))
        return conv1x1_bn_act(out, self.conv3, self.bn3, identity, enabled=FUSED_CONV1X1, split=SPLIT_RESGRAD and self.training)


class ResNet(nn.Module):
    def __init__(self, block, layers, num_classes=1000, groups=1, width_per_group=64, fused_bn=None,
                 zero_init_residual=False):
        super().__init__()
        self.inplanes = 64
        self.groups = groups
        self.base_width = width_per_group
        self.fused_bn = fused_bn
        self.conv1 = nn.Conv2d(3, 64, 7, stride=2, padding=3, bias=False)
        self.bn1 = BNAct(64, relu=True, fused=fused_bn)
        self.maxpool = nn.MaxPool2d(3, stride=2, padding=1)
        self.layer1 = self._make_layer(block, 64, layers[0])
        self.layer2 = self._make_layer(block, 128, layers[1], stride=2)
        self.layer3 = self._make_layer(block, 256, layers[2], stride=2)
        self.layer4 = self._make_layer(block, 512, layers[3], stride=2)
        self.avgpool = nn.AdaptiveAvgPool2d((1, 1))
        self.fc = nn.Linear(512 * block.expansion, num_classes)
        for m in self.modules():
            if isinstance(m, nn.Conv2d):
                nn.init.kaiming_normal_(m.weight, mode="fan_out", nonlinearity="relu")
            elif isinstance(m, nn.BatchNorm2d):
                nn.init.constant_(m.weight, 1.0)
                nn.init.constant_(m.bias, 0.0)
        if zero_init_residual:
            for m in self.modules():
                if isinstance(m, Bottleneck):
                    nn.init.constant_(m.bn3.weight, 0.0)
                elif isinstance(m, BasicBlock):
                    nn.init.constant_(m.bn2.weight, 0.0)

    def _make_layer(self, block, planes, blocks, stride=1):
        down = None
        if stride != 1 or self.inplanes != planes * block.expansion:
            down = _Downsample(self.inplanes, planes * block.expansion, stride, self.fused_bn)
        layers = [block(self.inplanes, planes, stride, down, self.groups, self.base_width, self.fused_bn)]
        self.inplanes = planes * block.expansion
        for _ in range(1, blocks):
            layers.append(block(self.inplanes, planes, groups=self.groups, base_width=self.base_width,
                                fused=self.fused_bn))
        return nn.Sequential(*layers)

    def forward(self, x):
        if self.training:
            begin_step(x.device)
        bn = self.bn1
        if STEM_GEMM and bn.training and torch.is_grad_enabled() and bn.fused is not False and (
                can_use_stem_gemm(x, self.conv1) or bn.fused == "emulate"):
            x = stem_conv_bn_relu_maxpool(x, self.conv1, bn, emulate=bn.fused == "emulate")
            x = self.layer4(self.layer3(self.layer2(self.layer1(x))))
            return self.fc(torch.flatten(self.avgpool(_pair(x)[0]), 1))
        nbt = bn.num_batches_tracked if (bn.training and bn.track_running_stats) else None
        x = bn_relu_maxpool(self.conv1(x), bn.weight, bn.bias, bn.running_mean, bn.running_var,
                            training=bn.training or not bn.track_running_stats, momentum=0.1 if bn.momentum is None else bn.momentum,
                            eps=bn.eps, fused=bn.fused, num_batches_tracked=nbt)
        x = self.layer4(self.layer3(self.layer2(self.layer1(x))))
        x = _pair(x)[0]
        return self.fc(torch.flatten(self.avgpool(x), 1))


def _factory(block, layers, **fixed):
    def make(num_classes=1000, fused_bn=None, **kw):
        return ResNet(block, layers, num_classes=num_classes, fused_bn=fused_bn, **fixed, **kw)
    return make


FACTORIES = {
    "resnet18": _factory(BasicBlock, [2, 2, 2, 2]),
    "resnet34": _factory(BasicBlock, [3, 4, 6, 3]),
    "resnet50": _factory(Bottleneck, [3, 4, 6, 3]),
    "resnet101": _factory(Bottleneck, [3, 4, 23, 3]),
    "resnet152": _factory(Bottleneck, [3, 8, 36, 3]),
    "resnext50_32x4d": _factory(Bottleneck, [3, 4, 6, 3], groups=32, width_per_group=4),
    "resnext101_32x8d": _factory(Bottleneck, [3, 4, 23, 3], groups=32, width_per_group=8),
    "resnext101_64x4d": _factory(Bottleneck, [3, 4, 23, 3], groups=64, width_per_group=4),
    "wide_resnet50_2": _factory(Bottleneck, [3, 4, 6, 3], width_per_group=128),
    "wide_resnet101_2": _factory(Bottleneck, [3, 4, 23, 3], width_per_group=128),
}
```

### pytorch_distributed_b200/ops/conv_bn.py

```python
from __future__ import annotations

import torch

from .bn_act import _BnActFn, _can_fuse, workspace


class _Conv1x1Stats(torch.autograd.Function):
    @staticmethod
    def forward(ctx, x, weight, stats):
        from .. import _ext
        _ext.note_launch(2)
        y = _ext.lib().conv1x1_bnstats(x, weight, stats)
        ctx.save_for_backward(x, weight)
        return y

    @staticmethod
    def backward(ctx, dy):
        x, weight = ctx.saved_tensors
        dy = dy.contiguous(memory_format=torch.channels_last)
        dx, dw, _ = torch.ops.aten.convolution_backward(dy, x, weight, None, (1, 1), (0, 0), (1, 1), False, (0, 0), 1,
                                                        (ctx.needs_input_grad[0], ctx.needs_input_grad[1], False))
        return dx, dw, None


def can_fuse_conv1x1(x, conv) -> bool:
    w = conv.weight
    return (x.is_cuda and x.dtype == torch.bfloat16 and w.dtype == torch.bfloat16 and x.dim() == 4
            and conv.kernel_size == (1, 1) and conv.stride == (1, 1) and conv.padding == (0, 0) and conv.groups == 1 and conv.bias is None
            and x.is_contiguous(memory_format=torch.channels_last) and x.size(1) % 64 == 0 and w.size(0) % 64 == 0
            and x.size(0) * x.size(2) * x.size(3) >= 128)


def conv1x1_bn_act(x, conv, bn, residual=None, enabled=True, split=False):
    training = bn.training or not bn.track_running_stats
    if not (enabled and training and can_fuse_conv1x1(x, conv) and bn.fused is not False):
        return bn(conv(x), residual, split) if split else bn(conv(x), residual)
    nc = conv.weight.size(0)
    ws = workspace(x.device)
    work, gen = ws.take(4 * nc)
    y = _Conv1x1Stats.apply(x, conv.weight, work[: 2 * nc])
    if not _can_fuse(y, bn.weight, residual, bn.running_mean):
        return bn(y, residual, split) if split else bn(y, residual)
    need_grad = torch.is_grad_enabled() and (y.requires_grad or bn.weight.requires_grad)
    nbt = bn.num_batches_tracked if (bn.training and bn.track_running_stats) else None
    out = _BnActFn.apply(y, residual, bn.weight, bn.bias, bn.running_mean, bn.running_var, nbt, True,
                         0.1 if bn.momentum is None else float(bn.momentum), float(bn.eps), bn.relu, need_grad, (work, gen),
                         bool(split and need_grad))
    if split and not isinstance(out, tuple):
        return out, out
    return out
```

Before: 6938 images/s.

## Fuse block-boundary BN-act with next conv1x1 and add masked dgrad GEMM

Adds a WGMMA/TMA dgrad GEMM kernel that fuses the residual-gradient add and ReLU mask into the 1x1 conv data-gradient epilogue, plus a masked BN backward entry point. The ResNet forward is restructured so each bottleneck's final BN+add+ReLU is fused with the next block's first 1x1 conv (with BN stats), deferring work across block boundaries. Shared TMA/WGMMA helpers move into a common header. This is meant to remove separate elementwise passes and activation round-trips through HBM, at the cost of more custom-kernel complexity and changed autograd structure.

```diff
diff --git a/pytorch_distributed_b200/_ext.py b/pytorch_distributed_b200/_ext.py
--- a/pytorch_distributed_b200/_ext.py
+++ b/pytorch_distributed_b200/_ext.py
@@ -12,8 +12,8 @@
 _NAME = "_C"
 _SO = os.path.join(_HERE, _NAME + ".so")
 _STAMP = os.path.join(_HERE, _NAME + ".hash")
-_SOURCES = ["bindings.cpp", "symm.cpp", "hvd_core.cpp", "collectives.cu", "optim.cu", "bn_act.cu", "data_ops.cu", "gemm_bnstats.cu", "stem_conv.cu",
-            "resample.cu"]
+_SOURCES = ["bindings.cpp", "symm.cpp", "hvd_core.cpp", "collectives.cu", "optim.cu", "bn_act.cu", "data_ops.cu", "gemm_bnstats.cu", "gemm_dgrad.cu",
+            "stem_conv.cu", "resample.cu"]
 _lock = threading.Lock()
 _mod = None
 _err = None
diff --git a/pytorch_distributed_b200/csrc/bindings.cpp b/pytorch_distributed_b200/csrc/bindings.cpp
--- a/pytorch_distributed_b200/csrc/bindings.cpp
+++ b/pytorch_distributed_b200/csrc/bindings.cpp
@@ -98,11 +98,13 @@
   m.def("bn_act_forward", &bn_act_forward);
   m.def("bn_act_backward", &bn_act_backward);
   m.def("bn_act_backward2", &bn_act_backward2);
+  m.def("bn_bwd_masked", &bn_bwd_masked);
   m.def("stem_forward", &stem_forward);
   m.def("stem_forward_pre", &stem_forward_pre);
   m.def("stem_backward", &stem_backward);
   m.def("stem_im2col", &stem_im2col);
   m.def("conv1x1_bnstats", &conv1x1_bnstats);
+  m.def("dgrad_mask", &dgrad_mask);
   m.def("normalize_nhwc", &normalize_nhwc);
   m.def("resample_normalize", &resample_normalize, py::arg("arena"), py::arg("n"), py::arg("out_h"), py::arg("out_w"), py::arg("max_rows"),
         py::arg("a"), py::arg("b"), py::arg("out_dtype"), py::arg("channels_last"));
diff --git a/pytorch_distributed_b200/csrc/bn_act.cu b/pytorch_distributed_b200/csrc/bn_act.cu
--- a/pytorch_distributed_b200/csrc/bn_act.cu
+++ b/pytorch_distributed_b200/csrc/bn_act.cu
@@ -603,6 +603,10 @@
 }
 
 template <typename T>
+static void apply_masked_impl(const at::Tensor& gin, const at::Tensor& x, const at::Tensor& saved, const at::Tensor& work, const at::Tensor& w,
+                              at::Tensor& dx, at::Tensor& dw, at::Tensor& db);
+
+template <typename T>
 static void bwd2_impl(const at::Tensor& dya, const at::Tensor& dyb, const at::Tensor& mask, const at::Tensor& x, const at::Tensor& saved,
                       at::Tensor& work, const at::Tensor& w, at::Tensor& g_out, at::Tensor& dx, at::Tensor& dw, at::Tensor& db, bool relu) {
   const Geometry g = geometry(x);
@@ -623,10 +627,55 @@
   else      bn_bwd_reduce_sum_kernel<T, false><<<rgrid, kBnThreads, g.smem, st>>>(ap, bp, mk, xp, sv, gp, pp, g.M, g.C, rpb);
   C10_CUDA_KERNEL_LAUNCH_CHECK();
   combine_partials(pp, rgrid, 2 * g.C, wk, st);
-  bn_bwd_apply_kernel<T, false, false><<<apply_grid(g), kBnThreads, 0, st>>>(gp, nullptr, xp, sv, wk, w.data_ptr(), wdtype(w),
-                                                                           reinterpret_cast<T*>(dx.data_ptr()), nullptr, dw.data_ptr(),
-                                                                           db.data_ptr(), g.M, g.C);
+  apply_masked_impl<T>(g_out, x, saved, work, w, dx, dw, db);
+}
+
+template <typename T>
+static void apply_masked_impl(const at::Tensor& gin, const at::Tensor& x, const at::Tensor& saved, const at::Tensor& work, const at::Tensor& w,
+                              at::Tensor& dx, at::Tensor& dw, at::Tensor& db) {
+  const Geometry g = geometry(x);
+  bn_bwd_apply_kernel<T, false, false><<<apply_grid(g), kBnThreads, 0, at::cuda::getCurrentCUDAStream()>>>(
+      reinterpret_cast<const T*>(gin.data_ptr()), nullptr, reinterpret_cast<const T*>(x.data_ptr()), saved.data_ptr<float>(),
+      work.data_ptr<float>(), w.data_ptr(), wdtype(w), reinterpret_cast<T*>(dx.data_ptr()), nullptr, dw.data_ptr(), db.data_ptr(), g.M, g.C);
   C10_CUDA_KERNEL_LAUNCH_CHECK();
+}
+
+template <typename T>
+static void bwd_masked_impl(const at::Tensor& gin, const at::Tensor& x, const at::Tensor& saved, at::Tensor& work, const at::Tensor& w,
+                            at::Tensor& dx, at::Tensor& dw, at::Tensor& db) {
+  const Geometry g = geometry(x);
+  cudaStream_t st = at::cuda::getCurrentCUDAStream();
+  int rpb;
+  const int rgrid = reduce_grid(g, &rpb, resident_ctas(bn_bwd_reduce_sum_kernel<T, true>, g.smem));
+  at::Tensor part = partials(x, rgrid, g.C);
+  float* pp = part.data_ptr<float>();
+  bn_bwd_reduce_kernel<T, false><<<rgrid, kBnThreads, g.smem, st>>>(reinterpret_cast<const T*>(gin.data_ptr()), nullptr,
+                                                                     reinterpret_cast<const T*>(x.data_ptr()), saved.data_ptr<float>(),
+                                                                     pp, g.M, g.C, rpb);
+  C10_CUDA_KERNEL_LAUNCH_CHECK();
+  combine_partials(pp, rgrid, 2 * g.C, work.data_ptr<float>(), st);
+  apply_masked_impl<T>(gin, x, saved, work, w, dx, dw, db);
+}
+
+std::vector<at::Tensor> bn_bwd_masked(const at::Tensor& g_in, const at::Tensor& x, const at::Tensor& weight, const at::Tensor& saved,
+                                      at::Tensor work) {
+  check_nhwc(x, "x");
+  const auto cl = at::MemoryFormat::ChannelsLast;
+  at::Tensor gin = g_in.is_contiguous(cl) ? g_in : g_in.contiguous(cl);
+  TORCH_CHECK(gin.scalar_type() == x.scalar_type() && gin.sizes() == x.sizes() && gin.device() == x.device(), "g must match x");
+  const int C = (int)x.size(1);
+  TORCH_CHECK(work.defined() && work.scalar_type() == at::kFloat && work.numel() >= 2 * C, "work buffer too small");
+  TORCH_CHECK(saved.defined() && saved.scalar_type() == at::kFloat && saved.numel() >= 2 * C, "saved statistics missing");
+  c10::cuda::CUDAGuard guard(x.device());
+  at::Tensor dx = at::empty_like(x, x.options().memory_format(cl));
+  at::Tensor dw = at::empty_like(weight), db = at::empty_like(weight);
+  switch (x.scalar_type()) {
+    case at::kBFloat16: bwd_masked_impl<__nv_bfloat16>(gin, x, saved, work, weight, dx, dw, db); break;
+    case at::kHalf: bwd_masked_impl<__half>(gin, x, saved, work, weight, dx, dw, db); break;
+    case at::kFloat: bwd_masked_impl<float>(gin, x, saved, work, weight, dx, dw, db); break;
+    default: TORCH_CHECK(false, "unsupported activation dtype");
+  }
+  return {dx, dw, db};
 }
 
 std::vector<at::Tensor> bn_act_backward2(const at::Tensor& dy_a_in, const at::Tensor& dy_b_in, const at::Tensor& x,
diff --git a/pytorch_distributed_b200/csrc/gemm_bnstats.cu b/pytorch_distributed_b200/csrc/gemm_bnstats.cu
--- a/pytorch_distributed_b200/csrc/gemm_bnstats.cu
+++ b/pytorch_distributed_b200/csrc/gemm_bnstats.cu
@@ -5,13 +5,9 @@
 
 #include "common.cuh"
 #include "host.h"
+#include "wgmma_tma.cuh"
 
 namespace ptd {
-
-constexpr int kBlockM = 128;
-constexpr int kBlockK = 64;
-constexpr int kConsumerThreads = 256;
-constexpr int kGemmThreads = kConsumerThreads + 32;
 
 template <int BLOCK_N> struct GemmCfg {
   static constexpr int kStages = BLOCK_N == 256 ? 3 : 4;
@@ -21,68 +17,6 @@
   static constexpr int kStatFloats = 2 * 4 * 128;
   static constexpr int kSmem = 1024 + kStages * (kABytes + kBBytes) + kCBytes + kStatFloats * 4 + 2 * kStages * 8;
 };
-
-__device__ __forceinline__ uint32_t smem_u32(const void* p) { return (uint32_t)__cvta_generic_to_shared(p); }
-
-__device__ __forceinline__ void mbar_init(uint64_t* bar, uint32_t count) {
-  asm volatile("mbarrier.init.shared::cta.b64 [%0], %1;" ::"r"(smem_u32(bar)), "r"(count));
-}
-__device__ __forceinline__ void mbar_expect_tx(uint64_t* bar, uint32_t bytes) {
-  asm volatile("mbarrier.arrive.expect_tx.shared::cta.b64 _, [%0], %1;" ::"r"(smem_u32(bar)), "r"(bytes) : "memory");
-}
-__device__ __forceinline__ void mbar_arrive(uint64_t* bar) {
-  asm volatile("mbarrier.arrive.shared::cta.b64 _, [%0];" ::"r"(smem_u32(bar)) : "memory");
-}
-__device__ __forceinline__ void mbar_wait(uint64_t* bar, uint32_t parity) {
-  const uint32_t addr = smem_u32(bar);
-  uint32_t done, spins = 0;
-  do {
-    asm volatile("{\n\t.reg .pred p;\n\tmbarrier.try_wait.parity.shared::cta.b64 p, [%1], %2;\n\tselp.u32 %0, 1, 0, p;\n\t}"
-                 : "=r"(done) : "r"(addr), "r"(parity) : "memory");
-    if (!done && ++spins > (1u << 24)) __trap();
-  } while (!done);
-}
-__device__ __forceinline__ void tma_load_2d(void* smem_dst, const CUtensorMap* map, uint64_t* bar, int c0, int c1) {
-  asm volatile("cp.async.bulk.tensor.2d.shared::cluster.global.mbarrier::complete_tx::bytes [%0], [%1, {%3, %4}], [%2];"
-               ::"r"(smem_u32(smem_dst)), "l"(map), "r"(smem_u32(bar)), "r"(c0), "r"(c1) : "memory");
-}
-__device__ __forceinline__ void named_barrier(int id, int threads) {
-  asm volatile("bar.sync %0, %1;" ::"r"(id), "r"(threads) : "memory");
-}
-
-__device__ __forceinline__ uint64_t gmma_desc(const void* smem_tile) {
-  const uint64_t addr = (uint64_t)(smem_u32(smem_tile) >> 4) & 0x3FFFull;
-  return addr | (1ull << 16) | ((uint64_t)(1024 >> 4) << 32) | (1ull << 62);
-}
-
-#define PTD_F8(i) "+f"(d[i]), "+f"(d[i + 1]), "+f"(d[i + 2]), "+f"(d[i + 3]), "+f"(d[i + 4]), "+f"(d[i + 5]), "+f"(d[i + 6]), "+f"(d[i + 7])
-
-__device__ __forceinline__ void wgmma_n64(float* d, uint64_t adesc, uint64_t bdesc, int accumulate) {
-  asm volatile(
-      "{\n\t.reg .pred p;\n\tsetp.ne.b32 p, %34, 0;\n\t"
-      "wgmma.mma_async.sync.aligned.m64n64k16.f32.bf16.bf16 "
-      "{%0, %1, %2, %3, %4, %5, %6, %7, %8, %9, %10, %11, %12, %13, %14, %15, "
-      "%16, %17, %18, %19, %20, %21, %22, %23, %24, %25, %26, %27, %28, %29, %30, %31}, %32, %33, p, 1, 1, 0, 0;\n\t}"
-      : PTD_F8(0), PTD_F8(8), PTD_F8(16), PTD_F8(24)
-      : "l"(adesc), "l"(bdesc), "r"(accumulate));
-}
-__device__ __forceinline__ void wgmma_n128(float* d, uint64_t adesc, uint64_t bdesc, int accumulate) {
-  asm volatile(
-      "{\n\t.reg .pred p;\n\tsetp.ne.b32 p, %66, 0;\n\t"
-      "wgmma.mma_async.sync.aligned.m64n128k16.f32.bf16.bf16 "
-      "{%0, %1, %2, %3, %4, %5, %6, %7, %8, %9, %10, %11, %12, %13, %14, %15, "
-      "%16, %17, %18, %19, %20, %21, %22, %23, %24, %25, %26, %27, %28, %29, %30, %31, "
-      "%32, %33, %34, %35, %36, %37, %38, %39, %40, %41, %42, %43, %44, %45, %46, %47, "
-      "%48, %49, %50, %51, %52, %53, %54, %55, %56, %57, %58, %59, %60, %61, %62, %63}, %64, %65, p, 1, 1, 0, 0;\n\t}"
-      : PTD_F8(0), PTD_F8(8), PTD_F8(16), PTD_F8(24), PTD_F8(32), PTD_F8(40), PTD_F8(48), PTD_F8(56)
-      : "l"(adesc), "l"(bdesc), "r"(accumulate));
-}
-#undef PTD_F8
-
-template <int N> __device__ __forceinline__ void fence_regs(float (&d)[N]) {
-#pragma unroll
-  for (int i = 0; i < N; ++i) asm volatile("" : "+f"(d[i])::"memory");
-}
 
 template <int BLOCK_N>
 __global__ void __launch_bounds__(kGemmThreads, 1) gemm_bnstats_kernel(const __grid_constant__ CUtensorMap tmap_a,
@@ -206,32 +140,6 @@
   }
 }
 
-typedef CUresult (*EncodeTiledFn)(CUtensorMap*, CUtensorMapDataType, cuuint32_t, void*, const cuuint64_t*, const cuuint64_t*, const cuuint32_t*,
-                                  const cuuint32_t*, CUtensorMapInterleave, CUtensorMapSwizzle, CUtensorMapL2promotion, CUtensorMapFloatOOBfill);
-
-static EncodeTiledFn encode_fn() {
-  static EncodeTiledFn fn = nullptr;
-  if (!fn) {
-    void* p = nullptr;
-    cudaDriverEntryPointQueryResult q;
-    TORCH_CHECK(cudaGetDriverEntryPoint("cuTensorMapEncodeTiled", &p, cudaEnableDefault, &q) == cudaSuccess && p, "cuTensorMapEncodeTiled not found");
-    fn = reinterpret_cast<EncodeTiledFn>(p);
-  }
-  return fn;
-}
-
-static CUtensorMap make_map(const void* ptr, int64_t rows, int64_t cols, int box_rows, CUtensorMapL2promotion promo) {
-  CUtensorMap m;
-  cuuint64_t dims[2] = {(cuuint64_t)cols, (cuuint64_t)rows};
-  cuuint64_t strides[1] = {(cuuint64_t)cols * 2};
-  cuuint32_t box[2] = {(cuuint32_t)kBlockK, (cuuint32_t)box_rows};
-  cuuint32_t estr[2] = {1, 1};
-  CUresult r = encode_fn()(&m, CU_TENSOR_MAP_DATA_TYPE_BFLOAT16, 2, const_cast<void*>(ptr), dims, strides, box, estr, CU_TENSOR_MAP_INTERLEAVE_NONE,
-                           CU_TENSOR_MAP_SWIZZLE_128B, promo, CU_TENSOR_MAP_FLOAT_OOB_FILL_NONE);
-  TORCH_CHECK(r == CUDA_SUCCESS, "cuTensorMapEncodeTiled failed: ", (int)r);
-  return m;
-}
-
 template <int BLOCK_N>
 static void launch_gemm(const at::Tensor& a, const at::Tensor& b, at::Tensor& c, at::Tensor& gsum, int M, int N, int K) {
   constexpr int smem = GemmCfg<BLOCK_N>::kSmem;
diff --git a/pytorch_distributed_b200/csrc/gemm_dgrad.cu b/pytorch_distributed_b200/csrc/gemm_dgrad.cu
--- /dev/null
+++ b/pytorch_distributed_b200/csrc/gemm_dgrad.cu
@@ -0,0 +1,204 @@
+#include <ATen/cuda/CUDAContext.h>
+#include <c10/cuda/CUDAGuard.h>
+#include <cuda.h>
+#include <torch/extension.h>
+
+#include "common.cuh"
+#include "host.h"
+#include "wgmma_tma.cuh"
+
+namespace ptd {
+
+template <int BLOCK_N> struct DgradCfg {
+  static constexpr int kStages = 4;
+  static constexpr int kABytes = kBlockM * kBlockK * 2;
+  static constexpr int kBBytes = BLOCK_N * kBlockK * 2;
+  static constexpr int kCBytes = kBlockM * BLOCK_N * 2;
+  static constexpr int kGroups = BLOCK_N / 8;
+  static constexpr int kRowStep = 128 / kGroups;
+  static constexpr int kRowsPerThread = 64 / kRowStep;
+  static constexpr int kSmem = 1024 + kStages * (kABytes + kBBytes) + kCBytes + 2 * kStages * 8;
+};
+
+__device__ __forceinline__ void unpack8(const V4& v, float (&f)[8]) {
+  float2 t;
+  t = Wire<__nv_bfloat16>::unpack2(v.x); f[0] = t.x; f[1] = t.y;
+  t = Wire<__nv_bfloat16>::unpack2(v.y); f[2] = t.x; f[3] = t.y;
+  t = Wire<__nv_bfloat16>::unpack2(v.z); f[4] = t.x; f[5] = t.y;
+  t = Wire<__nv_bfloat16>::unpack2(v.w); f[6] = t.x; f[7] = t.y;
+}
+
+template <int BLOCK_N>
+__global__ void __launch_bounds__(kGemmThreads, 1) dgrad_mask_kernel(const __grid_constant__ CUtensorMap tmap_a,
+                                                                    const __grid_constant__ CUtensorMap tmap_b,
+                                                                    const __grid_constant__ CUtensorMap tmap_g,
+                                                                    const __nv_bfloat16* __restrict__ dyb,
+                                                                    const uint8_t* __restrict__ mask, int M, int N, int K,
+                                                                    int m_tiles, int n_tiles, int ctas_per_n) {
+  using Cfg = DgradCfg<BLOCK_N>;
+  constexpr int kStages = Cfg::kStages;
+  constexpr int kInstN = BLOCK_N >= 128 ? 128 : 64;
+  constexpr int kBoxes = BLOCK_N / 64;
+  extern __shared__ uint8_t smem_raw[];
+  uint8_t* smem = reinterpret_cast<uint8_t*>((reinterpret_cast<uintptr_t>(smem_raw) + 1023) & ~(uintptr_t)1023);
+  uint8_t* smem_a = smem;
+  uint8_t* smem_b = smem_a + kStages * Cfg::kABytes;
+  uint8_t* smem_c = smem_b + kStages * Cfg::kBBytes;
+  uint64_t* full_bar = reinterpret_cast<uint64_t*>(smem_c + Cfg::kCBytes);
+  uint64_t* empty_bar = full_bar + kStages;
+
+  const int warp = threadIdx.x >> 5, lane = threadIdx.x & 31;
+  const int n_tile = blockIdx.x % n_tiles;
+  const int m_first = blockIdx.x / n_tiles;
+  const int n0 = n_tile * BLOCK_N;
+  const int num_kb = K / kBlockK;
+
+  if (threadIdx.x == 0) {
+    for (int s = 0; s < kStages; ++s) { mbar_init(&full_bar[s], 1); mbar_init(&empty_bar[s], kConsumerThreads / 32); }
+    asm volatile("fence.mbarrier_init.release.cluster;" ::: "memory");
+  }
+  __syncthreads();
+
+  if (warp == kConsumerThreads / 32) {
+    if (lane == 0) {
+      asm volatile("prefetch.tensormap [%0];" ::"l"(&tmap_a) : "memory");
+      asm volatile("prefetch.tensormap [%0];" ::"l"(&tmap_b) : "memory");
+      uint32_t it = 0;
+      for (int mt = m_first; mt < m_tiles; mt += ctas_per_n) {
+        for (int kb = 0; kb < num_kb; ++kb, ++it) {
+          const int s = it % kStages;
+          mbar_wait(&empty_bar[s], ((it / kStages) & 1) ^ 1);
+          mbar_expect_tx(&full_bar[s], Cfg::kABytes + Cfg::kBBytes);
+          tma_load_2d(smem_a + s * Cfg::kABytes, &tmap_a, &full_bar[s], kb * kBlockK, mt * kBlockM);
+          tma_load_2d(smem_b + s * Cfg::kBBytes, &tmap_b, &full_bar[s], kb * kBlockK, n0);
+        }
+      }
+    }
+    return;
+  }
+
+  const int wg = warp >> 2, t = threadIdx.x & 127, w = warp & 3;
+  uint8_t* stg = smem_c + wg * (Cfg::kCBytes / 2);
+  float acc[BLOCK_N / 2] = {};
+  const int r0 = 16 * w + (lane >> 2);
+  const int cg = t % Cfg::kGroups, rp = t / Cfg::kGroups;
+  uint8_t* stg_box = stg + (cg >> 3) * 8192;
+  const int gran = cg & 7;
+  const int c0 = n0 + cg * 8;
+
+  uint32_t it = 0;
+  for (int mt = m_first; mt < m_tiles; mt += ctas_per_n) {
+    const int64_t row0 = (int64_t)mt * kBlockM + wg * 64;
+    V4 bv[Cfg::kRowsPerThread];
+    uint32_t mb[Cfg::kRowsPerThread];
+#pragma unroll
+    for (int i = 0; i < Cfg::kRowsPerThread; ++i) {
+      const int64_t row = row0 + rp + i * Cfg::kRowStep;
+      if (row < M) {
+        bv[i] = ld_stream(dyb + row * N + c0);
+        mb[i] = mask[row * (N >> 3) + (c0 >> 3)];
+      } else {
+        bv[i] = V4{0u, 0u, 0u, 0u};
+        mb[i] = 0u;
+      }
+    }
+    for (int kb = 0; kb < num_kb; ++kb, ++it) {
+      const int st = it % kStages;
+      mbar_wait(&full_bar[st], (it / kStages) & 1);
+      const uint64_t adesc = gmma_desc(smem_a + st * Cfg::kABytes + wg * 64 * 128);
+      const uint64_t bdesc = gmma_desc(smem_b + st * Cfg::kBBytes);
+      fence_regs(acc);
+      asm volatile("wgmma.fence.sync.aligned;" ::: "memory");
+#pragma unroll
+      for (int k = 0; k < kBlockK / 16; ++k) {
+#pragma unroll
+        for (int h = 0; h < BLOCK_N / kInstN; ++h) {
+          if constexpr (kInstN == 128) wgmma_n128(acc + h * 64, adesc + 2 * k, bdesc + h * 8 * kInstN + 2 * k, (kb | k) != 0);
+          else wgmma_n64(acc + h * 32, adesc + 2 * k, bdesc + h * 8 * kInstN + 2 * k, (kb | k) != 0);
+        }
+      }
+      asm volatile("wgmma.commit_group.sync.aligned;" ::: "memory");
+      asm volatile("wgmma.wait_group.sync.aligned 0;" ::: "memory");
+      fence_regs(acc);
+      if (lane == 0) mbar_arrive(&empty_bar[st]);
+    }
+
+    if (t == 0) asm volatile("cp.async.bulk.wait_group.read 0;" ::: "memory");
+    named_barrier(1 + wg, 128);
+#pragma unroll
+    for (int j = 0; j < BLOCK_N / 8; ++j) {
+      uint8_t* box = stg + (j >> 3) * 8192 + (lane & 3) * 4;
+      const int g = j & 7;
+      *reinterpret_cast<uint32_t*>(box + r0 * 128 + ((g ^ (r0 & 7)) << 4)) = Wire<__nv_bfloat16>::pack2(acc[4 * j], acc[4 * j + 1]);
+      *reinterpret_cast<uint32_t*>(box + (r0 + 8) * 128 + ((g ^ (r0 & 7)) << 4)) =
+          Wire<__nv_bfloat16>::pack2(acc[4 * j + 2], acc[4 * j + 3]);
+    }
+    named_barrier(1 + wg, 128);
+
+#pragma unroll
+    for (int i = 0; i < Cfg::kRowsPerThread; ++i) {
+      const int r = rp + i * Cfg::kRowStep;
+      V4* sp = reinterpret_cast<V4*>(stg_box + r * 128 + ((gran ^ (r & 7)) << 4));
+      float d[8], e[8];
+      unpack8(*sp, d);
+      unpack8(bv[i], e);
+#pragma unroll
+      for (int k = 0; k < 8; ++k) d[k] = (mb[i] >> k) & 1u ? __bfloat162float(__float2bfloat16_rn(d[k] + e[k])) : 0.f;
+      using W = Wire<__nv_bfloat16>;
+      *sp = V4{W::pack2(d[0], d[1]), W::pack2(d[2], d[3]), W::pack2(d[4], d[5]), W::pack2(d[6], d[7])};
+    }
+    asm volatile("fence.proxy.async.shared::cta;" ::: "memory");
+    named_barrier(1 + wg, 128);
+    if (t == 0) {
+#pragma unroll
+      for (int b = 0; b < kBoxes; ++b) tma_store_2d(&tmap_g, stg + b * 8192, n0 + b * 64, mt * kBlockM + wg * 64);
+      asm volatile("cp.async.bulk.commit_group;" ::: "memory");
+    }
+  }
+  if (t == 0) asm volatile("cp.async.bulk.wait_group 0;" ::: "memory");
+}
+
+template <int BLOCK_N>
+static void launch_dgrad(const at::Tensor& dz, const at::Tensor& wt, at::Tensor& g, const at::Tensor& dyb, const at::Tensor& mask, int M,
+                         int N, int K) {
+  constexpr int smem = DgradCfg<BLOCK_N>::kSmem;
+  static bool configured[64] = {};
+  const int dev = dz.get_device();
+  if (!configured[dev & 63]) {
+    C10_CUDA_CHECK(cudaFuncSetAttribute(dgrad_mask_kernel<BLOCK_N>, cudaFuncAttributeMaxDynamicSharedMemorySize, smem));
+    configured[dev & 63] = true;
+  }
+  const CUtensorMap ma = make_map(dz.data_ptr(), M, K, kBlockM, CU_TENSOR_MAP_L2_PROMOTION_L2_256B);
+  const CUtensorMap mb = make_map(wt.data_ptr(), N, K, BLOCK_N, CU_TENSOR_MAP_L2_PROMOTION_L2_256B);
+  const CUtensorMap mg = make_map(g.data_ptr(), M, N, 64, CU_TENSOR_MAP_L2_PROMOTION_NONE);
+  const int m_tiles = (M + kBlockM - 1) / kBlockM, n_tiles = N / BLOCK_N;
+  const int sms = at::cuda::getCurrentDeviceProperties()->multiProcessorCount;
+  const int ctas_per_n = std::max(1, std::min(m_tiles, sms / n_tiles));
+  dgrad_mask_kernel<BLOCK_N><<<ctas_per_n * n_tiles, kGemmThreads, smem, at::cuda::getCurrentCUDAStream()>>>(
+      ma, mb, mg, reinterpret_cast<const __nv_bfloat16*>(dyb.data_ptr()), mask.data_ptr<uint8_t>(), M, N, K, m_tiles, n_tiles, ctas_per_n);
+  C10_CUDA_KERNEL_LAUNCH_CHECK();
+}
+
+at::Tensor dgrad_mask(const at::Tensor& dz_in, const at::Tensor& weight, const at::Tensor& dy_b_in, const at::Tensor& mask) {
+  const auto cl = at::MemoryFormat::ChannelsLast;
+  at::Tensor dz = dz_in.is_contiguous(cl) ? dz_in : dz_in.contiguous(cl);
+  at::Tensor dyb = dy_b_in.is_contiguous(cl) ? dy_b_in : dy_b_in.contiguous(cl);
+  TORCH_CHECK(dz.is_cuda() && dz.dim() == 4 && dz.scalar_type() == at::kBFloat16, "dgrad_mask: dz must be a bf16 CUDA tensor");
+  const int64_t M64 = dz.size(0) * dz.size(2) * dz.size(3);
+  const int K = (int)dz.size(1), N = (int)weight.size(1);
+  TORCH_CHECK(weight.dim() == 4 && weight.size(0) == K && weight.size(2) == 1 && weight.size(3) == 1 && weight.scalar_type() == at::kBFloat16,
+              "dgrad_mask: weight must be [K, N, 1, 1] bf16");
+  TORCH_CHECK(dyb.scalar_type() == at::kBFloat16 && dyb.dim() == 4 && dyb.size(0) == dz.size(0) && dyb.size(1) == N && dyb.size(2) == dz.size(2) &&
+                  dyb.size(3) == dz.size(3) && dyb.device() == dz.device(), "dgrad_mask: dy_b must be [B, N, H, W] bf16 matching dz");
+  TORCH_CHECK(K % kBlockK == 0 && N % 64 == 0 && M64 < (int64_t)1 << 31, "dgrad_mask: unsupported shape");
+  TORCH_CHECK(mask.is_cuda() && mask.scalar_type() == at::kByte && mask.numel() == M64 * N / 8, "dgrad_mask: mask must hold one bit per element");
+  c10::cuda::CUDAGuard guard(dz.device());
+  at::Tensor wt = weight.reshape({K, N}).t().contiguous();
+  at::Tensor g = at::empty_like(dyb, dyb.options().memory_format(cl));
+  const int M = (int)M64;
+  if (N % 128 == 0) launch_dgrad<128>(dz, wt, g, dyb, mask, M, N, K);
+  else launch_dgrad<64>(dz, wt, g, dyb, mask, M, N, K);
+  return g;
+}
+
+}
diff --git a/pytorch_distributed_b200/csrc/host.h b/pytorch_distributed_b200/csrc/host.h
--- a/pytorch_distributed_b200/csrc/host.h
+++ b/pytorch_distributed_b200/csrc/host.h
@@ -48,6 +48,8 @@
 std::vector<at::Tensor> bn_act_backward2(const at::Tensor& dy_a, const at::Tensor& dy_b, const at::Tensor& x,
                                          const c10::optional<at::Tensor>& mask, const at::Tensor& weight, const at::Tensor& saved, bool relu,
                                          at::Tensor work);
+std::vector<at::Tensor> bn_bwd_masked(const at::Tensor& g, const at::Tensor& x, const at::Tensor& weight, const at::Tensor& saved,
+                                      at::Tensor work);
 
 std::vector<at::Tensor> stem_forward(const at::Tensor& x, const at::Tensor& weight, const at::Tensor& bias, at::Tensor running_mean,
                                      at::Tensor running_var, c10::optional<at::Tensor> num_batches_tracked, bool training, double momentum,
@@ -59,6 +61,7 @@
                                       const at::Tensor& saved, at::Tensor work);
 
 at::Tensor conv1x1_bnstats(const at::Tensor& x, const at::Tensor& weight, at::Tensor gsum);
+at::Tensor dgrad_mask(const at::Tensor& dz, const at::Tensor& weight, const at::Tensor& dy_b, const at::Tensor& mask);
 
 at::Tensor stem_im2col(const at::Tensor& x);
 
diff --git a/pytorch_distributed_b200/csrc/wgmma_tma.cuh b/pytorch_distributed_b200/csrc/wgmma_tma.cuh
--- /dev/null
+++ b/pytorch_distributed_b200/csrc/wgmma_tma.cuh
@@ -0,0 +1,107 @@
+#pragma once
+#include <cuda.h>
+#include <cuda_runtime.h>
+#include <stdint.h>
+
+#include <ATen/ATen.h>
+
+namespace ptd {
+
+constexpr int kBlockM = 128;
+constexpr int kBlockK = 64;
+constexpr int kConsumerThreads = 256;
+constexpr int kGemmThreads = kConsumerThreads + 32;
+
+__device__ __forceinline__ uint32_t smem_u32(const void* p) { return (uint32_t)__cvta_generic_to_shared(p); }
+
+__device__ __forceinline__ void mbar_init(uint64_t* bar, uint32_t count) {
+  asm volatile("mbarrier.init.shared::cta.b64 [%0], %1;" ::"r"(smem_u32(bar)), "r"(count));
+}
+__device__ __forceinline__ void mbar_expect_tx(uint64_t* bar, uint32_t bytes) {
+  asm volatile("mbarrier.arrive.expect_tx.shared::cta.b64 _, [%0], %1;" ::"r"(smem_u32(bar)), "r"(bytes) : "memory");
+}
+__device__ __forceinline__ void mbar_arrive(uint64_t* bar) {
+  asm volatile("mbarrier.arrive.shared::cta.b64 _, [%0];" ::"r"(smem_u32(bar)) : "memory");
+}
+__device__ __forceinline__ void mbar_wait(uint64_t* bar, uint32_t parity) {
+  const uint32_t addr = smem_u32(bar);
+  uint32_t done, spins = 0;
+  do {
+    asm volatile("{\n\t.reg .pred p;\n\tmbarrier.try_wait.parity.shared::cta.b64 p, [%1], %2;\n\tselp.u32 %0, 1, 0, p;\n\t}"
+                 : "=r"(done) : "r"(addr), "r"(parity) : "memory");
+    if (!done && ++spins > (1u << 24)) __trap();
+  } while (!done);
+}
+__device__ __forceinline__ void tma_load_2d(void* smem_dst, const CUtensorMap* map, uint64_t* bar, int c0, int c1) {
+  asm volatile("cp.async.bulk.tensor.2d.shared::cluster.global.mbarrier::complete_tx::bytes [%0], [%1, {%3, %4}], [%2];"
+               ::"r"(smem_u32(smem_dst)), "l"(map), "r"(smem_u32(bar)), "r"(c0), "r"(c1) : "memory");
+}
+__device__ __forceinline__ void tma_store_2d(const CUtensorMap* map, const void* smem_src, int c0, int c1) {
+  asm volatile("cp.async.bulk.tensor.2d.global.shared::cta.bulk_group [%0, {%2, %3}], [%1];"
+               ::"l"(map), "r"(smem_u32(smem_src)), "r"(c0), "r"(c1) : "memory");
+}
+__device__ __forceinline__ void named_barrier(int id, int threads) {
+  asm volatile("bar.sync %0, %1;" ::"r"(id), "r"(threads) : "memory");
+}
+
+__device__ __forceinline__ uint64_t gmma_desc(const void* smem_tile) {
+  const uint64_t addr = (uint64_t)(smem_u32(smem_tile) >> 4) & 0x3FFFull;
+  return addr | (1ull << 16) | ((uint64_t)(1024 >> 4) << 32) | (1ull << 62);
+}
+
+#define PTD_F8(i) "+f"(d[i]), "+f"(d[i + 1]), "+f"(d[i + 2]), "+f"(d[i + 3]), "+f"(d[i + 4]), "+f"(d[i + 5]), "+f"(d[i + 6]), "+f"(d[i + 7])
+
+__device__ __forceinline__ void wgmma_n64(float* d, uint64_t adesc, uint64_t bdesc, int accumulate) {
+  asm volatile(
+      "{\n\t.reg .pred p;\n\tsetp.ne.b32 p, %34, 0;\n\t"
+      "wgmma.mma_async.sync.aligned.m64n64k16.f32.bf16.bf16 "
+      "{%0, %1, %2, %3, %4, %5, %6, %7, %8, %9, %10, %11, %12, %13, %14, %15, "
+      "%16, %17, %18, %19, %20, %21, %22, %23, %24, %25, %26, %27, %28, %29, %30, %31}, %32, %33, p, 1, 1, 0, 0;\n\t}"
+      : PTD_F8(0), PTD_F8(8), PTD_F8(16), PTD_F8(24)
+      : "l"(adesc), "l"(bdesc), "r"(accumulate));
+}
+__device__ __forceinline__ void wgmma_n128(float* d, uint64_t adesc, uint64_t bdesc, int accumulate) {
+  asm volatile(
+      "{\n\t.reg .pred p;\n\tsetp.ne.b32 p, %66, 0;\n\t"
+      "wgmma.mma_async.sync.aligned.m64n128k16.f32.bf16.bf16 "
+      "{%0, %1, %2, %3, %4, %5, %6, %7, %8, %9, %10, %11, %12, %13, %14, %15, "
+      "%16, %17, %18, %19, %20, %21, %22, %23, %24, %25, %26, %27, %28, %29, %30, %31, "
+      "%32, %33, %34, %35, %36, %37, %38, %39, %40, %41, %42, %43, %44, %45, %46, %47, "
+      "%48, %49, %50, %51, %52, %53, %54, %55, %56, %57, %58, %59, %60, %61, %62, %63}, %64, %65, p, 1, 1, 0, 0;\n\t}"
+      : PTD_F8(0), PTD_F8(8), PTD_F8(16), PTD_F8(24), PTD_F8(32), PTD_F8(40), PTD_F8(48), PTD_F8(56)
+      : "l"(adesc), "l"(bdesc), "r"(accumulate));
+}
+#undef PTD_F8
+
+template <int N> __device__ __forceinline__ void fence_regs(float (&d)[N]) {
+#pragma unroll
+  for (int i = 0; i < N; ++i) asm volatile("" : "+f"(d[i])::"memory");
+}
+
+typedef CUresult (*EncodeTiledFn)(CUtensorMap*, CUtensorMapDataType, cuuint32_t, void*, const cuuint64_t*, const cuuint64_t*, const cuuint32_t*,
+                                  const cuuint32_t*, CUtensorMapInterleave, CUtensorMapSwizzle, CUtensorMapL2promotion, CUtensorMapFloatOOBfill);
+
+static inline EncodeTiledFn encode_fn() {
+  static EncodeTiledFn fn = nullptr;
+  if (!fn) {
+    void* p = nullptr;
+    cudaDriverEntryPointQueryResult q;
+    TORCH_CHECK(cudaGetDriverEntryPoint("cuTensorMapEncodeTiled", &p, cudaEnableDefault, &q) == cudaSuccess && p, "cuTensorMapEncodeTiled not found");
+    fn = reinterpret_cast<EncodeTiledFn>(p);
+  }
+  return fn;
+}
+
+static inline CUtensorMap make_map(const void* ptr, int64_t rows, int64_t cols, int box_rows, CUtensorMapL2promotion promo) {
+  CUtensorMap m;
+  cuuint64_t dims[2] = {(cuuint64_t)cols, (cuuint64_t)rows};
+  cuuint64_t strides[1] = {(cuuint64_t)cols * 2};
+  cuuint32_t box[2] = {(cuuint32_t)kBlockK, (cuuint32_t)box_rows};
+  cuuint32_t estr[2] = {1, 1};
+  CUresult r = encode_fn()(&m, CU_TENSOR_MAP_DATA_TYPE_BFLOAT16, 2, const_cast<void*>(ptr), dims, strides, box, estr, CU_TENSOR_MAP_INTERLEAVE_NONE,
+                           CU_TENSOR_MAP_SWIZZLE_128B, promo, CU_TENSOR_MAP_FLOAT_OOB_FILL_NONE);
+  TORCH_CHECK(r == CUDA_SUCCESS, "cuTensorMapEncodeTiled failed: ", (int)r);
+  return m;
+}
+
+}
diff --git a/pytorch_distributed_b200/models/resnet.py b/pytorch_distributed_b200/models/resnet.py
--- a/pytorch_distributed_b200/models/resnet.py
+++ b/pytorch_distributed_b200/models/resnet.py
@@ -4,7 +4,7 @@
 import torch.nn as nn
 
 from ..ops.bn_act import begin_step, bn_act
-from ..ops.conv_bn import conv1x1_bn_act
+from ..ops.conv_bn import _apply_bn, bn_act_conv1x1, can_fuse_bn_conv1x1, can_fuse_conv1x1, conv1x1_bn_act, conv1x1_stats
 from ..ops.stem import bn_relu_maxpool
 from ..ops.stem_conv import can_use_stem_gemm, stem_conv_bn_relu_maxpool
 
@@ -12,10 +12,23 @@
 FUSED_CONV1X1 = _os.environ.get("PTD_FUSED_CONV1X1", "1") == "1"
 SPLIT_RESGRAD = _os.environ.get("PTD_SPLIT_RESGRAD", "1") == "1"
 STEM_GEMM = _os.environ.get("PTD_STEM_GEMM", "1") == "1"
+FUSED_DGRAD = _os.environ.get("PTD_FUSED_DGRAD", "1") == "1"
 
 
 def _pair(x):
     return x if isinstance(x, tuple) else (x, x)
+
+
+class _Pending(tuple):
+    """A Bottleneck output whose last BNAct is not applied yet: (z, pre, residual, bn) - the pre-BN conv3 output, its
+    GEMM-reduced statistics, the residual and the BNAct.  The next block applies it together with its own conv1."""
+
+
+def _dgrad_fusion(x, bn, conv, residual):
+    emulate = bn.fused == "emulate"
+    use = (FUSED_CONV1X1 and bool(FUSED_DGRAD) and emulate == (FUSED_DGRAD == "emulate")
+           and can_fuse_bn_conv1x1(x, bn, conv, residual))
+    return use, emulate
 
 
 class BNAct(nn.BatchNorm2d):
@@ -87,11 +100,30 @@
         self.stride = stride
 
     def forward(self, x):
-        x, skip = _pair(x)
+        return self._run(x)
+
+    def _run(self, x, defer=False):
+        split = SPLIT_RESGRAD and self.training
+        if isinstance(x, _Pending):
+            z, pre, res, bn = x
+            use, emu = _dgrad_fusion(z, bn, self.conv1, res)
+            if use:
+                skip, z1, pre1 = bn_act_conv1x1(z, bn, self.conv1, res, pre, emulate=emu)
+                out = _apply_bn(z1, self.bn1, None, False, pre1)
+            else:
+                x, skip = _pair(_apply_bn(z, bn, res, split, pre))
+                out = conv1x1_bn_act(x, self.conv1, self.bn1, enabled=FUSED_CONV1X1)
+        else:
+            x, skip = _pair(x)
+            out = conv1x1_bn_act(x, self.conv1, self.bn1, enabled=FUSED_CONV1X1)
         identity = skip if self.downsample is None else self.downsample(skip)
-        out = conv1x1_bn_act(x, self.conv1, self.bn1, enabled=FUSED_CONV1X1)
         out = self.bn2(self.conv2(out))
-        return conv1x1_bn_act(out, self.conv3, self.bn3, identity, enabled=FUSED_CONV1X1, split=SPLIT_RESGRAD and self.training)
+        emu = self.bn3.fused == "emulate"
+        if (defer and split and FUSED_CONV1X1 and emu == (FUSED_DGRAD == "emulate") and self.bn3.relu and self.bn3.fused is not False
+                and can_fuse_conv1x1(out, self.conv3, emu)):
+            z3, pre3 = conv1x1_stats(out, self.conv3, emu)
+            return _Pending((z3, pre3, identity, self.bn3))
+        return conv1x1_bn_act(out, self.conv3, self.bn3, identity, enabled=FUSED_CONV1X1, split=split)
 
 
 class ResNet(nn.Module):
@@ -142,15 +174,26 @@
         if STEM_GEMM and bn.training and torch.is_grad_enabled() and bn.fused is not False and (
                 can_use_stem_gemm(x, self.conv1) or bn.fused == "emulate"):
             x = stem_conv_bn_relu_maxpool(x, self.conv1, bn, emulate=bn.fused == "emulate")
-            x = self.layer4(self.layer3(self.layer2(self.layer1(x))))
+            x = self._layers(x)
             return self.fc(torch.flatten(self.avgpool(_pair(x)[0]), 1))
         nbt = bn.num_batches_tracked if (bn.training and bn.track_running_stats) else None
         x = bn_relu_maxpool(self.conv1(x), bn.weight, bn.bias, bn.running_mean, bn.running_var,
                             training=bn.training or not bn.track_running_stats, momentum=0.1 if bn.momentum is None else bn.momentum,
                             eps=bn.eps, fused=bn.fused, num_batches_tracked=nbt)
-        x = self.layer4(self.layer3(self.layer2(self.layer1(x))))
+        x = self._layers(x)
         x = _pair(x)[0]
         return self.fc(torch.flatten(self.avgpool(x), 1))
+
+
+    def _layers(self, x):
+        layers = (self.layer1, self.layer2, self.layer3, self.layer4)
+        blocks = [b for layer in layers for b in layer]
+        if not (FUSED_DGRAD and FUSED_CONV1X1 and SPLIT_RESGRAD and self.training and torch.is_grad_enabled()
+                and all(type(b) is Bottleneck for b in blocks)):
+            return self.layer4(self.layer3(self.layer2(self.layer1(x))))
+        for i, b in enumerate(blocks):
+            x = b._run(x, defer=i + 1 < len(blocks))
+        return x
 
 
 def _factory(block, layers, **fixed):
diff --git a/pytorch_distributed_b200/ops/conv_bn.py b/pytorch_distributed_b200/ops/conv_bn.py
--- a/pytorch_distributed_b200/ops/conv_bn.py
+++ b/pytorch_distributed_b200/ops/conv_bn.py
@@ -2,7 +2,7 @@
 
 import torch
 
-from .bn_act import _BnActFn, _can_fuse, workspace
+from .bn_act import _BnActFn, _can_fuse, _Emu, workspace
 
 
 class _Conv1x1Stats(torch.autograd.Function):
@@ -23,29 +23,115 @@
         return dx, dw, None
 
 
-def can_fuse_conv1x1(x, conv) -> bool:
+def can_fuse_conv1x1(x, conv, emulate=False) -> bool:
     w = conv.weight
-    return (x.is_cuda and x.dtype == torch.bfloat16 and w.dtype == torch.bfloat16 and x.dim() == 4
+    return ((emulate or (x.is_cuda and x.dtype == torch.bfloat16 and w.dtype == torch.bfloat16)) and x.dim() == 4
             and conv.kernel_size == (1, 1) and conv.stride == (1, 1) and conv.padding == (0, 0) and conv.groups == 1 and conv.bias is None
             and x.is_contiguous(memory_format=torch.channels_last) and x.size(1) % 64 == 0 and w.size(0) % 64 == 0
             and x.size(0) * x.size(2) * x.size(3) >= 128)
+
+
+def _apply_bn(y, bn, residual, split, pre):
+    if not _can_fuse(y, bn.weight, residual, bn.running_mean, emulate=bn.fused == "emulate"):
+        return bn(y, residual, split) if split else bn(y, residual)
+    need_grad = torch.is_grad_enabled() and (y.requires_grad or bn.weight.requires_grad)
+    nbt = bn.num_batches_tracked if (bn.training and bn.track_running_stats) else None
+    out = _BnActFn.apply(y, residual, bn.weight, bn.bias, bn.running_mean, bn.running_var, nbt, True,
+                         0.1 if bn.momentum is None else float(bn.momentum), float(bn.eps), bn.relu, need_grad, pre,
+                         bool(split and need_grad))
+    if split and not isinstance(out, tuple):
+        return out, out
+    return out
+
+
+def conv1x1_stats(x, conv, emulate=False):
+    nc = conv.weight.size(0)
+    work, gen = workspace(x.device).take(4 * nc)
+    if emulate:
+        return _EmuGemm.conv1x1_bnstats(x, conv.weight, work[: 2 * nc]), (work, gen)
+    return _Conv1x1Stats.apply(x, conv.weight, work[: 2 * nc]), (work, gen)
 
 
 def conv1x1_bn_act(x, conv, bn, residual=None, enabled=True, split=False):
     training = bn.training or not bn.track_running_stats
     if not (enabled and training and can_fuse_conv1x1(x, conv) and bn.fused is not False):
         return bn(conv(x), residual, split) if split else bn(conv(x), residual)
+    y, pre = conv1x1_stats(x, conv)
+    return _apply_bn(y, bn, residual, split, pre)
+
+
+class _EmuGemm(_Emu):
+
+    @staticmethod
+    def conv1x1_bnstats(x, weight, gsum):
+        n = weight.size(0)
+        y = (_Emu._rows(x).float() @ weight.reshape(n, -1).float().t()).to(x.dtype)
+        gsum[:n] += y.detach().float().sum(0)
+        gsum[n:2 * n] += (y.detach().float() ** 2).sum(0)
+        b, _, h, w = x.shape
+        return y.reshape(b, h, w, n).permute(0, 3, 1, 2)
+
+    @staticmethod
+    def dgrad_mask(dz, weight, dy_b, mask):
+        k, c = weight.size(0), weight.size(1)
+        d = (_Emu._rows(dz).float() @ weight.reshape(k, c).float()).to(dy_b.dtype).float()
+        d = (d + _Emu._rows(dy_b).float()).to(dy_b.dtype).float()
+        return _Emu._like(d * _Emu._unpack(mask, d.size(0), c), dy_b)
+
+    @staticmethod
+    def bn_bwd_masked(g, x, weight, saved, work):
+        dx, dw, db = _Emu._bwd_from_g(_Emu._rows(g).float(), x, weight, saved)
+        return dx, dw, db
+
+
+class _BnActConv1x1Fn(torch.autograd.Function):
+
+    @staticmethod
+    def forward(ctx, x, residual, weight, bias, running_mean, running_var, nbt, momentum, eps, pre, conv_weight, stats, emulate):
+        from .. import _ext
+        K = _EmuGemm if emulate else _ext.lib()
+        nc = x.size(1)
+        work, gen = pre
+        _ext.note_launch(3)
+        y, saved, mask = K.bn_act_forward(x, residual, weight, bias, running_mean, running_var, nbt, True, momentum, eps, True, True,
+                                          work[: 2 * nc], True)
+        z = K.conv1x1_bnstats(y, conv_weight, stats)
+        ctx.save_for_backward(x, mask, weight, saved, y, conv_weight)
+        ctx.work, ctx.gen, ctx.ws = work[2 * nc:], gen, workspace(x.device)
+        ctx.emulate = emulate
+        return y, z
+
+    @staticmethod
+    def backward(ctx, d_skip, dz):
+        from .. import _ext
+        x, mask, weight, saved, y, conv_weight = ctx.saved_tensors
+        K = _EmuGemm if ctx.emulate else _ext.lib()
+        work = ctx.work
+        if ctx.gen != -1 and ctx.gen != ctx.ws.generation:
+            work = torch.zeros(2 * x.size(1), dtype=torch.float32, device=x.device)
+        dz = dz.contiguous(memory_format=torch.channels_last)
+        if ctx.emulate:
+            dw_conv = torch.nn.grad.conv2d_weight(y.float(), conv_weight.shape, dz.float()).to(conv_weight.dtype)
+        else:
+            _, dw_conv, _ = torch.ops.aten.convolution_backward(dz, y, conv_weight, None, (1, 1), (0, 0), (1, 1), False, (0, 0), 1,
+                                                                (False, True, False))
+        _ext.note_launch(4)
+        g = K.dgrad_mask(dz, conv_weight, d_skip, mask)
+        dx, dgamma, dbeta = K.bn_bwd_masked(g, x, weight, saved, work)
+        return (dx, g, dgamma, dbeta) + (None,) * 6 + (dw_conv, None, None)
+
+
+def bn_act_conv1x1(x, bn, conv, residual, pre, emulate=False):
     nc = conv.weight.size(0)
-    ws = workspace(x.device)
-    work, gen = ws.take(4 * nc)
-    y = _Conv1x1Stats.apply(x, conv.weight, work[: 2 * nc])
-    if not _can_fuse(y, bn.weight, residual, bn.running_mean):
-        return bn(y, residual, split) if split else bn(y, residual)
-    need_grad = torch.is_grad_enabled() and (y.requires_grad or bn.weight.requires_grad)
-    nbt = bn.num_batches_tracked if (bn.training and bn.track_running_stats) else None
-    out = _BnActFn.apply(y, residual, bn.weight, bn.bias, bn.running_mean, bn.running_var, nbt, True,
-                         0.1 if bn.momentum is None else float(bn.momentum), float(bn.eps), bn.relu, need_grad, (work, gen),
-                         bool(split and need_grad))
-    if split and not isinstance(out, tuple):
-        return out, out
-    return out
+    zwork, zgen = workspace(x.device).take(4 * nc)
+    nbt = bn.num_batches_tracked if bn.track_running_stats else None
+    y, z = _BnActConv1x1Fn.apply(x, residual, bn.weight, bn.bias, bn.running_mean, bn.running_var, nbt,
+                                 0.1 if bn.momentum is None else float(bn.momentum), float(bn.eps), pre, conv.weight, zwork[: 2 * nc],
+                                 emulate)
+    return y, z, (zwork, zgen)
+
+
+def can_fuse_bn_conv1x1(x, bn, conv, residual) -> bool:
+    emulate = bn.fused == "emulate"
+    return (bn.training and bn.relu and bn.fused is not False and residual is not None and torch.is_grad_enabled()
+            and can_fuse_conv1x1(x, conv, emulate) and _can_fuse(x, bn.weight, residual, bn.running_mean, emulate=emulate))
```

Result: faster. 7113 images/s, median of 6 (+2.5%).
